# edwardyang12/Dex-NERF

Hardware: AMD Instinct MI355X
Metric: rays/sec (64+128 samples) + PSNR vs ref, 400x400 scene (higher is better)
Workload: dtype bf16; 1 GPU; C2 render: 400x400 rays/step/GPU, 64 coarse + 128 fine samples, coarse+fine FlexibleNeRFModel D8/W256/skip4 + viewdirs, PE L=10/4, 20 Dex thresholds, validation mode (det. resampling, no noise)

## Files before the change

### dex-nerf_amd/csrc/api.cpp

```cpp
#include <cstdlib>
#include <cstring>
#include <utility>
#include <vector>

#include "dn_common.h"
#include "composite_body.h"
#include "dn_rng.h"

namespace dn {

static thread_local char g_err[512] = "";

void set_error(const char* fmt, ...) {
  va_list ap;
  va_start(ap, fmt);
  vsnprintf(g_err, sizeof(g_err), fmt, ap);
  va_end(ap);
}

int ensure_big_lds(const void* kernel) {
  int dev = 0;
  if (hipGetDevice(&dev) != hipSuccess) dev = 0;
  static thread_local std::vector<std::pair<const void*, int>> done;
  for (const auto& kd : done)
    if (kd.first == kernel && kd.second == dev) return 0;
  hipError_t e = hipFuncSetAttribute(kernel, hipFuncAttributeMaxDynamicSharedMemorySize, 160 * 1024);
  if (e != hipSuccess) { set_error("hipFuncSetAttribute(device %d): %s", dev, hipGetErrorString(e)); return -static_cast<int>(e); }
  done.emplace_back(kernel, dev);
  return 0;
}

int device_cus() {
  constexpr int kMaxDev = 64;
  static thread_local int cache[kMaxDev] = {0};
  int dev = 0;
  if (hipGetDevice(&dev) != hipSuccess || dev < 0 || dev >= kMaxDev) return 256;
  if (cache[dev] == 0) {
    int cus = 256;
    if (hipDeviceGetAttribute(&cus, hipDeviceAttributeMultiprocessorCount, dev) != hipSuccess || cus <= 0) cus = 256;
    cache[dev] = cus;
  }
  return cache[dev];
}

static size_t align256(size_t v) { return (v + 255) & ~static_cast<size_t>(255); }

struct Workspace {
  float *z_c, *rf_c, *w_c, *z_f, *rf_f, *g_rf;
  unsigned* absmax_part;
  unsigned* status;
  size_t bytes;
};

static Workspace carve(void* base, int64_t n, int nc, int nf, bool train = false) {
  Workspace w{};
  size_t off = 0;
  auto take = [&](size_t floats) {
    float* p = base ? reinterpret_cast<float*>(static_cast<char*>(base) + off) : nullptr;
    off += align256(floats * sizeof(float));
    return p;
  };
  w.z_c = take(static_cast<size_t>(n) * nc);
  w.rf_c = take(static_cast<size_t>(n) * nc * 4);
  w.w_c = take(static_cast<size_t>(n) * nc);
  if (nf > 0) {
    w.z_f = take(static_cast<size_t>(n) * (nc + nf));
    w.rf_f = take(static_cast<size_t>(n) * (nc + nf) * 4);
  }
  if (train) w.g_rf = take(static_cast<size_t>(n) * (nc + nf) * 4);
  if (train) w.absmax_part = reinterpret_cast<unsigned*>(take(static_cast<size_t>((n + 3) / 4)));
  w.status = reinterpret_cast<unsigned*>(take(64));
  w.bytes = off;
  return w;
}

}

using namespace dn;

extern "C" int dn_abi_version(void) { return DN_ABI_VERSION; }

extern "C" const char* dn_last_error(void) { return g_err; }

extern "C" size_t dn_render_workspace_bytes(int64_t n_rays, int num_coarse, int num_fine) {
  if (n_rays < 0 || num_coarse < 1 || num_fine < 0) return 0;
  return carve(nullptr, n_rays, num_coarse, num_fine).bytes;
}

extern "C" int dn_render_rays(const dn_mlp_desc* desc_coarse, const void* packed_coarse, const dn_mlp_desc* desc_fine,
                              const void* packed_fine, int precision, const float* rays, int ray_stride,
                              int64_t n_rays, int num_coarse, int num_fine, int lindisp, float noise_std,
                              int white_background, const float* h_m_thres, int n_thres, const float* t_rand,
                              const float* noise_c, const float* u, const float* noise_f, float* rgb_c,
                              float* depth_c, float* acc_c, float* rgb_f, float* depth_f, float* acc_f, float* dex_f,
                              void* workspace, dn_stream_t stream) {
  if (n_rays == 0) return 0;
  DN_REQUIRE(desc_coarse && packed_coarse && rays && workspace && n_rays >= 0, "dn_render_rays: bad arguments");
  DN_REQUIRE(num_fine == 0 || (desc_fine && packed_fine), "dn_render_rays: fine pass requested without a fine net");
  DN_REQUIRE((reinterpret_cast<uintptr_t>(workspace) & 255) == 0, "dn_render_rays: workspace must be 256-byte aligned");
  if (n_rays == 0) return 0;
  Workspace w = carve(workspace, n_rays, num_coarse, num_fine);
  int rc;
  {
    hipError_t e = hipMemsetAsync(w.status, 0, 256, as_stream(stream));
    if (e != hipSuccess) { set_error("dn_render_rays: hipMemsetAsync: %s", hipGetErrorString(e)); return -static_cast<int>(e); }
  }
  if ((rc = dn_coarse_depths(rays, ray_stride, n_rays, num_coarse, lindisp, t_rand, w.z_c, stream))) return rc;
  const bool fine = num_fine > 0;
  DN_REQUIRE(n_thres >= 0 && n_thres <= kMaxThres, "dn_render_rays: at most %d Dex thresholds", kMaxThres);
  auto comp_for = [&](float* rgb, float* acc, float* weights, float* depth, float* dex, int k) {
    CompParams c{};
    c.rgb = rgb; c.acc = acc; c.weights = weights; c.depth = depth; c.dex = dex; c.disp = nullptr;
    c.nonfinite = w.status; c.n_rays = n_rays; c.n_thres = k; c.white = white_background;
    for (int i = 0; i < kMaxThres; ++i) c.th.m[i] = (i < k) ? h_m_thres[i] : 0.0f;
    return c;
  };
  const bool may_fuse = !(noise_std > 0.0f);
  int done = 0;
  {
    const CompParams c = comp_for(rgb_c, acc_c, w.w_c, depth_c, fine ? nullptr : dex_f, fine ? 0 : n_thres);
    if ((rc = run_network_flagged(desc_coarse, precision, packed_coarse, nullptr, nullptr, rays, ray_stride, w.z_c, n_rays,
                                  num_coarse, w.rf_c, w.status + 1, stream, (may_fuse && rgb_c) ? &c : nullptr, &done)))
      return rc;
  }
  if (!done && (rc = volume_render_counting(w.rf_c, w.z_c, rays + 3, ray_stride, noise_c, noise_std, white_background, h_m_thres,
                                            fine ? 0 : n_thres, n_rays, num_coarse, rgb_c, nullptr, acc_c, w.w_c, depth_c,
                                            fine ? nullptr : dex_f, w.status, stream)))
    return rc;
  if (!fine) return 0;
  if ((rc = dn_fine_depths(w.z_c, w.w_c, u, n_rays, num_coarse, num_fine, w.z_f, nullptr, stream))) return rc;
  {
    const CompParams c = comp_for(rgb_f, acc_f, nullptr, depth_f, dex_f, n_thres);
    if ((rc = run_network_flagged(desc_fine, precision, packed_fine, nullptr, nullptr, rays, ray_stride, w.z_f, n_rays,
                                  num_coarse + num_fine, w.rf_f, w.status + 1, stream, (may_fuse && rgb_f) ? &c : nullptr, &done)))
      return rc;
  }
  if (done) return 0;
  return volume_render_counting(w.rf_f, w.z_f, rays + 3, ray_stride, noise_f, noise_std, white_background, h_m_thres, n_thres,
                                n_rays, num_coarse + num_fine, rgb_f, nullptr, acc_f, nullptr, depth_f, dex_f, w.status, stream);
}

extern "C" size_t dn_render_train_workspace_bytes(int64_t n_rays, int num_coarse, int num_fine) {
  if (n_rays < 0 || num_coarse < 1 || num_fine < 0) return 0;
  return carve(nullptr, n_rays, num_coarse, num_fine, true).bytes;
}

extern "C" int dn_render_rays_train(const dn_mlp_desc* desc_coarse, const void* packed_coarse, const dn_mlp_desc* desc_fine,
                                    const void* packed_fine, int precision, const float* rays, int ray_stride,
                                    int64_t n_rays, int num_coarse, int num_fine, int lindisp, float noise_std,
                                    int white_background, const float* h_m_thres, int n_thres, const float* t_rand,
                                    const float* noise_c, const float* u, const float* noise_f, float* rgb_c,
                                    float* depth_c, float* acc_c, float* rgb_f, float* depth_f, float* acc_f, float* dex_f,
                                    void* workspace, void* act_c, void* masks_c, void* act_f, void* masks_f,
                                    const uint32_t* rng_state, int perturb, dn_stream_t stream) {
  if (n_rays == 0) return 0;
  DN_REQUIRE(desc_coarse && packed_coarse && rays && workspace && act_c && masks_c && n_rays >= 0, "dn_render_rays_train: bad arguments");
  DN_REQUIRE(num_fine == 0 || (desc_fine && packed_fine && act_f && masks_f), "dn_render_rays_train: fine pass requested without a fine net / its buffers");
  DN_REQUIRE((reinterpret_cast<uintptr_t>(workspace) & 255) == 0, "dn_render_rays_train: workspace must be 256-byte aligned");
  Workspace w = carve(workspace, n_rays, num_coarse, num_fine, true);
  int rc;
  const uint32_t* rng_perturb = perturb ? rng_state : nullptr;
  if ((rc = coarse_depths_rng(rays, ray_stride, n_rays, num_coarse, lindisp, t_rand, w.z_c, rng_perturb, stream))) return rc;
  if ((rc = dn_run_network_train(desc_coarse, precision, packed_coarse, nullptr, nullptr, rays, ray_stride, w.z_c, n_rays,
                                 num_coarse, w.rf_c, act_c, masks_c, stream)))
    return rc;
  const bool fine = num_fine > 0;
  if ((rc = volume_render_counting(w.rf_c, w.z_c, rays + 3, ray_stride, noise_c, noise_std, white_background, h_m_thres,
                                   fine ? 0 : n_thres, n_rays, num_coarse, rgb_c, nullptr, acc_c, w.w_c, depth_c,
                                   fine ? nullptr : dex_f, nullptr, stream, rng_state, kRngStreamNoiseCoarse)))
    return rc;
  if (!fine) return 0;
  if ((rc = fine_depths_rng(w.z_c, w.w_c, u, n_rays, num_coarse, num_fine, w.z_f, nullptr, rng_perturb, stream))) return rc;
  if ((rc = dn_run_network_train(desc_fine, precision, packed_fine, nullptr, nullptr, rays, ray_stride, w.z_f, n_rays,
                                 num_coarse + num_fine, w.rf_f, act_f, masks_f, stream)))
    return rc;
  return volume_render_counting(w.rf_f, w.z_f, rays + 3, ray_stride, noise_f, noise_std, white_background, h_m_thres, n_thres,
                                n_rays, num_coarse + num_fine, rgb_f, nullptr, acc_f, nullptr, depth_f, dex_f, nullptr, stream,
                                rng_state, kRngStreamNoiseFine);
}

extern "C" int dn_render_rays_backward_ws(const dn_mlp_desc* desc_coarse, const void* packed_bwd_coarse,
                                          const dn_mlp_desc* desc_fine, const void* packed_bwd_fine, int precision,
                                          const float* rays, int ray_stride, int64_t n_rays, int num_coarse, int num_fine,
                                          float noise_std, int white_background, const float* noise_c, const float* noise_f,
                                          const float* g_rgb_c, const float* g_depth_c, const float* g_acc_c,
                                          const float* g_rgb_f, const float* g_depth_f, const float* g_acc_f, void* workspace,
                                          const void* act_c, const void* masks_c, void* grads_c, const void* act_f,
                                          const void* masks_f, void* grads_f, float* const* h_dW_c, float* const* h_db_c,
                                          float* const* h_dW_f, float* const* h_db_f, int nets, const uint32_t* rng_state,
                                          void* wg_scratch, size_t wg_scratch_bytes, dn_stream_t stream) {
  if (n_rays == 0) return 0;
  DN_REQUIRE(rays && workspace && n_rays >= 0 && (nets & ~3) == 0 && (wg_scratch != nullptr || wg_scratch_bytes == 0), "dn_render_rays_backward: bad arguments");
  DN_REQUIRE((reinterpret_cast<uintptr_t>(workspace) & 255) == 0, "dn_render_rays_backward: workspace must be 256-byte aligned");
  Workspace w = carve(workspace, n_rays, num_coarse, num_fine, true);
  int rc;
  const bool pair_wgrad = nets == 3 && num_fine > 0 && desc_coarse && desc_fine && std::memcmp(desc_coarse, desc_fine, sizeof(dn_mlp_desc)) == 0 &&
                          weight_grad_pair_fits(*desc_fine);
  auto half = [&](const dn_mlp_desc* desc, const void* packed_bwd, const float* rf, const float* z, int samples,
                  const float* noise, const float* g_rgb, const float* g_depth, const float* g_acc, const void* act,
                  const void* masks, void* grads, float* const* h_dW, float* const* h_db, uint32_t noise_stream) -> int {
    DN_REQUIRE(desc && packed_bwd && act && masks && grads && h_dW && h_db, "dn_render_rays_backward: a network's buffers are missing");
    const int64_t n_parts = (n_rays + 3) / 4;
    unsigned* parts = (precision == DN_PREC_BF16_S8 && s8_scale_is_per_launch() && n_parts <= 4096 && std::getenv("DEXNERF_S8_ABSMAX_KERNEL") == nullptr)
                          ? w.absmax_part : nullptr;
    if ((rc = volume_render_backward_rng(rf, z, rays + 3, ray_stride, noise, noise_std, white_background, n_rays, samples,
                                         g_rgb, g_depth, g_acc, nullptr, nullptr, w.g_rf, rng_state, noise_stream, stream, parts)))
      return rc;
    const int64_t n_points = n_rays * samples;
    if ((rc = mlp_backward_data_partials(desc, precision, packed_bwd, w.g_rf, masks, n_points, grads, parts, static_cast<int>(parts ? n_parts : 0), stream))) return rc;
    if (pair_wgrad) return 0;
    return dn_mlp_weight_grad_all_ws(desc, precision, act, grads, n_points, h_dW, h_db, wg_scratch, wg_scratch_bytes, stream);
  };
  if ((nets & 2) && num_fine > 0) {
    if ((rc = half(desc_fine, packed_bwd_fine, w.rf_f, w.z_f, num_coarse + num_fine, noise_f, g_rgb_f, g_depth_f, g_acc_f,
                   act_f, masks_f, grads_f, h_dW_f, h_db_f, kRngStreamNoiseFine)))
      return rc;
  }
  if (nets & 1) {
    if ((rc = half(desc_coarse, packed_bwd_coarse, w.rf_c, w.z_c, num_coarse, noise_c, g_rgb_c, g_depth_c, g_acc_c, act_c,
                   masks_c, grads_c, h_dW_c, h_db_c, kRngStreamNoiseCoarse)))
      return rc;
  }
  if (pair_wgrad)
    return dn_mlp_weight_grad_pair_ws(desc_fine, precision, act_f, grads_f, n_rays * (num_coarse + num_fine), h_dW_f, h_db_f, act_c, grads_c,
                                      n_rays * num_coarse, h_dW_c, h_db_c, wg_scratch, wg_scratch_bytes, stream);
  return 0;
}

extern "C" int dn_render_rays_backward(const dn_mlp_desc* desc_coarse, const void* packed_bwd_coarse,
                                       const dn_mlp_desc* desc_fine, const void* packed_bwd_fine, int precision,
                                       const float* rays, int ray_stride, int64_t n_rays, int num_coarse, int num_fine,
                                       float noise_std, int white_background, const float* noise_c, const float* noise_f,
                                       const float* g_rgb_c, const float* g_depth_c, const float* g_acc_c,
                                       const float* g_rgb_f, const float* g_depth_f, const float* g_acc_f, void* workspace,
                                       const void* act_c, const void* masks_c, void* grads_c, const void* act_f,
                                       const void* masks_f, void* grads_f, float* const* h_dW_c, float* const* h_db_c,
                                       float* const* h_dW_f, float* const* h_db_f, int nets, const uint32_t* rng_state,
                                       dn_stream_t stream) {
  return dn_render_rays_backward_ws(desc_coarse, packed_bwd_coarse, desc_fine, packed_bwd_fine, precision, rays, ray_stride, n_rays, num_coarse,
                                    num_fine, noise_std, white_background, noise_c, noise_f, g_rgb_c, g_depth_c, g_acc_c, g_rgb_f, g_depth_f,
                                    g_acc_f, workspace, act_c, masks_c, grads_c, act_f, masks_f, grads_f, h_dW_c, h_db_c, h_dW_f, h_db_f, nets,
                                    rng_state, nullptr, 0, stream);
}
```

### dex-nerf_amd/csrc/dn_common.h

```cpp
#pragma once
#include <hip/hip_runtime.h>
#include <cstdarg>
#include <cstdint>
#include <cstdio>

#include "../../include/dexnerf_hip.h"

namespace dn {

constexpr int kWave = 64;

void set_error(const char* fmt, ...);

inline hipStream_t as_stream(dn_stream_t s) { return reinterpret_cast<hipStream_t>(s); }

inline int check_launch(const char* what) {
  hipError_t e = hipGetLastError();
  if (e != hipSuccess) {
    set_error("%s: %s", what, hipGetErrorString(e));
    return -static_cast<int>(e);
  }
  return 0;
}

int ensure_big_lds(const void* kernel);
int device_cus();

int volume_render_counting(const float* rf, const float* z, const float* rd, int rd_stride, const float* noise, float noise_std,
                           int white_background, const float* h_m_thres, int n_thres, int64_t n_rays, int n_samples, float* rgb,
                           float* disp, float* acc, float* weights, float* depth, float* dex, unsigned* nonfinite,
                           dn_stream_t stream, const uint32_t* rng_state = nullptr, uint32_t rng_stream = 0);

bool weight_grad_pair_fits(const dn_mlp_desc& d);
struct CompParams;
int run_network_flagged(const dn_mlp_desc* desc, int precision, const void* packed, const float* pts, const float* viewdirs,
                        const float* rays, int ray_stride, const float* z_vals, int64_t n_rays, int samples_per_ray, float* out,
                        unsigned* range_flag, dn_stream_t stream, const CompParams* comp = nullptr, int* composited = nullptr);

int coarse_depths_rng(const float* rays, int ray_stride, int64_t n_rays, int num_coarse, int lindisp, const float* t_rand,
                      float* z_vals, const uint32_t* rng_state, dn_stream_t stream);
int fine_depths_rng(const float* z_coarse, const float* weights, const float* u, int64_t n_rays, int num_coarse, int num_fine,
                    float* z_fine, float* z_samples, const uint32_t* rng_state, dn_stream_t stream);
int volume_render_backward_rng(const float* rf, const float* z, const float* rd, int rd_stride, const float* noise, float noise_std,
                               int white_background, int64_t n_rays, int n_samples, const float* g_rgb, const float* g_depth,
                               const float* g_acc, const float* g_disp, const float* g_weights, float* g_rf,
                               const uint32_t* rng_state, uint32_t rng_stream, dn_stream_t stream, unsigned* absmax_part = nullptr);
int mlp_backward_data_partials(const dn_mlp_desc* desc, int precision, const void* packed_bwd, const float* g_out, const void* masks,
                               int64_t n_points, void* grads, const unsigned* partials, int n_partials, dn_stream_t stream);
bool s8_scale_is_per_launch();

#define DN_REQUIRE(cond, ...)     \
  do {                            \
    if (!(cond)) {                \
      dn::set_error(__VA_ARGS__); \
      return DN_E_INVAL;          \
    }                             \
  } while (0)

__device__ __forceinline__ int lane_id() { return threadIdx.x & 63; }

template <int CTRL>
__device__ __forceinline__ unsigned dpp_bits(unsigned v) {
  return static_cast<unsigned>(__builtin_amdgcn_update_dpp(0, static_cast<int>(v), CTRL, 0xF, 0xF, false));
}
constexpr int kDppXor1 = 0xB1, kDppXor2 = 0x4E, kDppHalfMirror = 0x141, kDppMirror = 0x140;

template <class Op>
__device__ __forceinline__ float wave_allreduce(float v, Op op) {
  auto f = [](unsigned b) { return __builtin_bit_cast(float, b); };
  auto u = [](float x) { return __builtin_bit_cast(unsigned, x); };
  v = op(v, f(dpp_bits<kDppXor1>(u(v))));
  v = op(v, f(dpp_bits<kDppXor2>(u(v))));
  v = op(v, f(dpp_bits<kDppHalfMirror>(u(v))));
  v = op(v, f(dpp_bits<kDppMirror>(u(v))));
  { const auto r = __builtin_amdgcn_permlane16_swap(u(v), u(v), false, false); v = op(f(r[0]), f(r[1])); }
  { const auto r = __builtin_amdgcn_permlane32_swap(u(v), u(v), false, false); v = op(f(r[0]), f(r[1])); }
  return v;
}

__device__ __forceinline__ float wave_sum(float v) { return wave_allreduce(v, [](float a, float b) { return a + b; }); }
__device__ __forceinline__ float wave_max(float v) { return wave_allreduce(v, [](float a, float b) { return fmaxf(a, b); }); }

__device__ __forceinline__ double wave_sum(double v) {
  auto mv = [](double x, auto step) {
    const unsigned long long b = __builtin_bit_cast(unsigned long long, x);
    const unsigned lo = step(static_cast<unsigned>(b)), hi = step(static_cast<unsigned>(b >> 32));
    return __builtin_bit_cast(double, (static_cast<unsigned long long>(hi) << 32) | lo);
  };
  v += mv(v, [](unsigned w) { return dpp_bits<kDppXor1>(w); });
  v += mv(v, [](unsigned w) { return dpp_bits<kDppXor2>(w); });
  v += mv(v, [](unsigned w) { return dpp_bits<kDppHalfMirror>(w); });
  v += mv(v, [](unsigned w) { return dpp_bits<kDppMirror>(w); });
  {
    const unsigned long long b = __builtin_bit_cast(unsigned long long, v);
    const auto lo = __builtin_amdgcn_permlane16_swap(static_cast<unsigned>(b), static_cast<unsigned>(b), false, false);
    const auto hi = __builtin_amdgcn_permlane16_swap(static_cast<unsigned>(b >> 32), static_cast<unsigned>(b >> 32), false, false);
    v = __builtin_bit_cast(double, (static_cast<unsigned long long>(hi[0]) << 32) | lo[0]) +
        __builtin_bit_cast(double, (static_cast<unsigned long long>(hi[1]) << 32) | lo[1]);
  }
  {
    const unsigned long long b = __builtin_bit_cast(unsigned long long, v);
    const auto lo = __builtin_amdgcn_permlane32_swap(static_cast<unsigned>(b), static_cast<unsigned>(b), false, false);
    const auto hi = __builtin_amdgcn_permlane32_swap(static_cast<unsigned>(b >> 32), static_cast<unsigned>(b >> 32), false, false);
    v = __builtin_bit_cast(double, (static_cast<unsigned long long>(hi[0]) << 32) | lo[0]) +
        __builtin_bit_cast(double, (static_cast<unsigned long long>(hi[1]) << 32) | lo[1]);
  }
  return v;
}

template <int CTRL, int ROW_MASK>
__device__ __forceinline__ double dpp_or_one(double v) {
  const unsigned long long b = __builtin_bit_cast(unsigned long long, v);
  const unsigned lo = static_cast<unsigned>(__builtin_amdgcn_update_dpp(0, static_cast<int>(static_cast<unsigned>(b)), CTRL, ROW_MASK, 0xF, false));
  const unsigned hi = static_cast<unsigned>(__builtin_amdgcn_update_dpp(0x3FF00000, static_cast<int>(static_cast<unsigned>(b >> 32)), CTRL, ROW_MASK, 0xF, false));
  return __builtin_bit_cast(double, (static_cast<unsigned long long>(hi) << 32) | lo);
}
__device__ __forceinline__ double wave_scan_mul(double v) {
  v *= dpp_or_one<0x111, 0xF>(v);
  v *= dpp_or_one<0x112, 0xF>(v);
  v *= dpp_or_one<0x114, 0xF>(v);
  v *= dpp_or_one<0x118, 0xF>(v);
  v *= dpp_or_one<0x142, 0xA>(v);
  v *= dpp_or_one<0x143, 0xC>(v);
  return v;
}
__device__ __forceinline__ double wave_shift_up1(double v, double first) {
  const unsigned long long b = __builtin_bit_cast(unsigned long long, v), f = __builtin_bit_cast(unsigned long long, first);
  const unsigned lo = static_cast<unsigned>(__builtin_amdgcn_update_dpp(static_cast<int>(static_cast<unsigned>(f)), static_cast<int>(static_cast<unsigned>(b)), 0x138, 0xF, 0xF, false));
  const unsigned hi = static_cast<unsigned>(__builtin_amdgcn_update_dpp(static_cast<int>(static_cast<unsigned>(f >> 32)), static_cast<int>(static_cast<unsigned>(b >> 32)), 0x138, 0xF, 0xF, false));
  return __builtin_bit_cast(double, (static_cast<unsigned long long>(hi) << 32) | lo);
}
__device__ __forceinline__ double wave_last(double v) {
  const unsigned long long b = __builtin_bit_cast(unsigned long long, v);
  const unsigned lo = static_cast<unsigned>(__builtin_amdgcn_readlane(static_cast<int>(static_cast<unsigned>(b)), 63));
  const unsigned hi = static_cast<unsigned>(__builtin_amdgcn_readlane(static_cast<int>(static_cast<unsigned>(b >> 32)), 63));
  return __builtin_bit_cast(double, (static_cast<unsigned long long>(hi) << 32) | lo);
}

__device__ __forceinline__ double wave_scan_add(double v) {
  const int l = lane_id();
#pragma unroll
  for (int o = 1; o < 64; o <<= 1) {
    double t = __shfl_up(v, o, 64);
    if (l >= o) v += t;
  }
  return v;
}

__device__ __forceinline__ float wave_scan_add(float v) {
  const int l = lane_id();
#pragma unroll
  for (int o = 1; o < 64; o <<= 1) {
    float t = __shfl_up(v, o, 64);
    if (l >= o) v += t;
  }
  return v;
}

__host__ __device__ __forceinline__ float linspace_elem(float start, float end, int steps, int i) {
  if (steps == 1) return start;
  const float step = (end - start) / static_cast<float>(steps - 1);
  return (i < steps / 2) ? fmaf(step, static_cast<float>(i), start)
                         : fmaf(-step, static_cast<float>(steps - 1 - i), end);
}

}
```

### dex-nerf_amd/csrc/mlp_device.h

```cpp
#pragma once
#include <cstdlib>
#include <utility>

#include "mlp_layout.h"

namespace dn {

typedef float f32x16 __attribute__((ext_vector_type(16)));
typedef float f32x4 __attribute__((ext_vector_type(4)));
typedef __bf16 bf16x8 __attribute__((ext_vector_type(8)));
typedef _Float16 f16x8 __attribute__((ext_vector_type(8)));

template <int N, class F, int... I>
__device__ __forceinline__ void static_for_impl(F&& f, std::integer_sequence<int, I...>) {
  (f(std::integral_constant<int, I>{}), ...);
}
template <int N, class F>
__device__ __forceinline__ void static_for(F&& f) {
  static_for_impl<N>(static_cast<F&&>(f), std::make_integer_sequence<int, N>{});
}

constexpr int kRingPhases = 5;
constexpr int kSlotBytes = kPhasePieces * kPieceBytes;
constexpr int kRingBytes = kRingPhases * kSlotBytes;
constexpr int kInRows = 10;

template <int BF16> struct Prec;
template <> struct Prec<1> {
  using BPiece = bf16x8;
  using Elem = __bf16;
  static constexpr int EPP = 8;
  static constexpr int PPT = 2;
};
template <> struct Prec<2> {
  using BPiece = f16x8;
  using Elem = _Float16;
  static constexpr int EPP = 8;
  static constexpr int PPT = 2;
};
template <> struct Prec<0> {
  using BPiece = f32x4;
  using Elem = float;
  static constexpr int EPP = 4;
  static constexpr int PPT = 4;
};
template <int BF16, int PT> constexpr int waves_of() { return (BF16 && PT == 1) ? 8 : 4; }

struct FwdParams {
  const char* packed;
  int bias_bytes;
  int total_pieces;
  int D;
  unsigned skip_mask;
  int use_viewdirs;
  int mode;
  const float* rays;
  int ray_stride;
  const float* z;
  const float* pts;
  const float* viewdirs;
  const float* enc;
  int enc_ld;
  long long n_points;
  int S;
  long long n_tiles;
  float* out;
  float fx[16];
  float fd[8];
  char* act;
  char* masks;
  int act_pieces, mask_words;
  int slot_xyz, slot_dir, slot_layer1, slot_trunk0, slot_feat, slot_dirout;
  int save8;
  unsigned* range_flag;
};

template <bool ASM_READS_, bool LEADER_DMA_, bool SCALAR_STATE_, int PREFETCH_>
struct PipeGeometry {
  static constexpr bool ASM_READS = ASM_READS_, LEADER_DMA = LEADER_DMA_, SCALAR_STATE = SCALAR_STATE_;
  static constexpr int PREFETCH = PREFETCH_;
};
template <int WAVES, class G>
struct PipeT {
  static constexpr int PER_WAVE = kPhasePieces / WAVES;
  char* ring;
  unsigned ring_addr;
  const char* wsrc;
  unsigned total_bytes;
  unsigned q_issue;
  unsigned slot_wr, slot_nxt;
  unsigned wave;
  unsigned pend_src, pend_dst;
  const char* rd_cur;
  const char* rd_nxt;
  unsigned lane16;
  f32x4 af[G::PREFETCH];
  unsigned rda_cur;
  unsigned slot_cur_base;
  f32x4 bias_nxt;

  __device__ __forceinline__ void dma_phase(unsigned src_off, unsigned dst_off, unsigned go) {
    const unsigned long long src_bits = reinterpret_cast<unsigned long long>(wsrc + src_off);
    const unsigned lo = __builtin_amdgcn_readfirstlane(static_cast<unsigned>(src_bits));
    const unsigned hi = __builtin_amdgcn_readfirstlane(static_cast<unsigned>(src_bits >> 32));
    const char* src = reinterpret_cast<const char*>((static_cast<unsigned long long>(hi) << 32) | lo);
    const unsigned lds = __builtin_amdgcn_readfirstlane(ring_addr + dst_off);
    go = __builtin_amdgcn_readfirstlane(go);
    unsigned keep;
    if constexpr (PER_WAVE == 2) {
      asm volatile(
          "s_cmp_lg_u32 %[go], 0\n\t"
          "s_cbranch_scc0 .Ldn_dma_skip%=\n\t"
          "s_mov_b32 %[keep], m0\n\t"
          "s_mov_b32 m0, %[lds]\n\t"
          "s_nop 1\n\t"
          "global_load_lds_dwordx4 %[voff], %[sbase]\n\t"
          "global_load_lds_dwordx4 %[voff], %[sbase] offset:1024\n\t"
          "s_mov_b32 m0, %[keep]\n"
          ".Ldn_dma_skip%=:"
          : [keep] "=&s"(keep)
          : [go] "s"(go), [lds] "s"(lds), [voff] "v"(lane16), [sbase] "s"(src)
          : "memory", "scc");
    } else {
      asm volatile(
          "s_cmp_lg_u32 %[go], 0\n\t"
          "s_cbranch_scc0 .Ldn_dma_skip%=\n\t"
          "s_mov_b32 %[keep], m0\n\t"
          "s_mov_b32 m0, %[lds]\n\t"
          "s_nop 1\n\t"
          "global_load_lds_dwordx4 %[voff], %[sbase]\n\t"
          "global_load_lds_dwordx4 %[voff], %[sbase] offset:1024\n\t"
          "global_load_lds_dwordx4 %[voff], %[sbase] offset:2048\n\t"
          "global_load_lds_dwordx4 %[voff], %[sbase] offset:3072\n\t"
          "s_mov_b32 m0, %[keep]\n"
          ".Ldn_dma_skip%=:"
          : [keep] "=&s"(keep)
          : [go] "s"(go), [lds] "s"(lds), [voff] "v"(lane16), [sbase] "s"(src)
          : "memory", "scc");
    }
  }

  __device__ __forceinline__ void advance_issue() {
    const unsigned who = wave;
    if constexpr (G::LEADER_DMA) {
      pend_src = q_issue + who * (2 * PER_WAVE * kPieceBytes);
      pend_dst = slot_wr * kSlotBytes + who * (2 * PER_WAVE * kPieceBytes);
    } else {
      pend_src = q_issue + who * (PER_WAVE * kPieceBytes);
      pend_dst = slot_wr * kSlotBytes + who * (PER_WAVE * kPieceBytes);
    }
    q_issue += kSlotBytes;
    if (q_issue >= total_bytes) q_issue = 0;
    slot_wr = (slot_wr + 1 == kRingPhases) ? 0 : slot_wr + 1;
    if constexpr (G::SCALAR_STATE) {
      q_issue = __builtin_amdgcn_readfirstlane(q_issue);
      slot_wr = __builtin_amdgcn_readfirstlane(slot_wr);
      pend_src = __builtin_amdgcn_readfirstlane(pend_src);
      pend_dst = __builtin_amdgcn_readfirstlane(pend_dst);
    }
  }

  __device__ __forceinline__ void issue_phase() {
    advance_issue();
    if constexpr (G::LEADER_DMA) {
      dma_phase(pend_src, pend_dst, wave < 4 ? 1u : 0u);
      dma_phase(pend_src + PER_WAVE * kPieceBytes, pend_dst + PER_WAVE * kPieceBytes, wave < 4 ? 1u : 0u);
    } else {
      dma_phase(pend_src, pend_dst, 1u);
    }
  }

  __device__ __forceinline__ void phase_begin() {
    static_assert(kRingPhases == 5, "the counted waits below assume two younger phases in flight");
    if constexpr (G::ASM_READS) {
      static_assert(!G::ASM_READS || PER_WAVE == 2, "the asm-read pipeline is the 8-wave geometry");
      if constexpr (G::LEADER_DMA) asm volatile("s_waitcnt vmcnt(8)" ::: "memory");
      else asm volatile("s_waitcnt vmcnt(4)" ::: "memory");
    } else {
      if constexpr (PER_WAVE == 2) asm volatile("s_waitcnt vmcnt(4) lgkmcnt(0)" ::: "memory");
      else asm volatile("s_waitcnt vmcnt(8) lgkmcnt(0)" ::: "memory");
    }
    __builtin_amdgcn_s_barrier();
    advance_issue();
    dma_phase(pend_src, pend_dst, (WAVES == 4 || wave < 4) ? 1u : 0u);
    slot_nxt = (slot_nxt + 1 == kRingPhases) ? 0 : slot_nxt + 1;
    if constexpr (G::ASM_READS) {
      rda_cur = slot_cur_base + lane16;
      slot_cur_base = __builtin_amdgcn_readfirstlane(ring_addr + slot_nxt * kSlotBytes);
    } else {
      rd_cur = rd_nxt;
      rd_nxt = ring + slot_nxt * kSlotBytes + lane16;
    }
  }

  __device__ __forceinline__ void mid_phase() {
    if constexpr (WAVES == 8 && G::LEADER_DMA) dma_phase(pend_src + PER_WAVE * kPieceBytes, pend_dst + PER_WAVE * kPieceBytes, wave < 4 ? 1u : 0u);
    else if constexpr (WAVES == 8) dma_phase(pend_src, pend_dst, wave >= 4 ? 1u : 0u);
  }

  template <bool EVEN>
  __device__ __forceinline__ void phase_begin2() {
    if constexpr (EVEN) {
      asm volatile("s_waitcnt vmcnt(0)" ::: "memory");
      __builtin_amdgcn_s_barrier();
      advance_issue();
      dma_phase(pend_src, pend_dst, wave < 4 ? 1u : 0u);
      dma_phase(pend_src + PER_WAVE * kPieceBytes, pend_dst + PER_WAVE * kPieceBytes, wave < 4 ? 1u : 0u);
    }
    slot_nxt = (slot_nxt + 1 == kRingPhases) ? 0 : slot_nxt + 1;
    rda_cur = slot_cur_base + lane16;
    slot_cur_base = __builtin_amdgcn_readfirstlane(ring_addr + slot_nxt * kSlotBytes);
  }
  template <bool EVEN>
  __device__ __forceinline__ void mid_phase2() {
    if constexpr (EVEN) {
      advance_issue();
      dma_phase(pend_src, pend_dst, wave < 4 ? 1u : 0u);
      dma_phase(pend_src + PER_WAVE * kPieceBytes, pend_dst + PER_WAVE * kPieceBytes, wave < 4 ? 1u : 0u);
    }
  }
  unsigned long long xs_src[2];
  unsigned xs_dst[2];
  template <int PERIOD>
  __device__ __forceinline__ void xs_period_begin() {
    static_assert(PERIOD == kPhasePieces || PERIOD == 2 * kPhasePieces, "barrier period: one or two phases");
    if constexpr (PERIOD == 2 * kPhasePieces) asm volatile("s_waitcnt vmcnt(0)" ::: "memory");
    else asm volatile("s_waitcnt vmcnt(8)" ::: "memory");
    __builtin_amdgcn_s_barrier();
#pragma unroll
    for (int h = 0; h < PERIOD / kPhasePieces; ++h) {
      advance_issue();
      const unsigned long long bits = reinterpret_cast<unsigned long long>(wsrc + pend_src);
      const unsigned lo = __builtin_amdgcn_readfirstlane(static_cast<unsigned>(bits));
      const unsigned hi = __builtin_amdgcn_readfirstlane(static_cast<unsigned>(bits >> 32));
      xs_src[h] = (static_cast<unsigned long long>(hi) << 32) | lo;
      xs_dst[h] = __builtin_amdgcn_readfirstlane(ring_addr + pend_dst);
    }
  }
  template <int PERIOD, int Q>
  __device__ __forceinline__ void xs_dma_step() {
    constexpr int STEPS = PERIOD / 8;
    constexpr int H = (Q % STEPS) / 2;
    constexpr int OFF = (Q % 2) * 2048;
    unsigned keep;
    asm volatile(
        "s_cmp_lg_u32 %[wave], %[who]\n\t"
        "s_cbranch_scc1 .Ldn_xs_skip%=\n\t"
        "s_mov_b32 %[keep], m0\n\t"
        "s_mov_b32 m0, %[lds]\n\t"
        "s_nop 1\n\t"
        "global_load_lds_dwordx4 %[voff], %[sbase] offset:%[o0]\n\t"
        "global_load_lds_dwordx4 %[voff], %[sbase] offset:%[o1]\n\t"
        "s_mov_b32 m0, %[keep]\n"
        ".Ldn_xs_skip%=:"
        : [keep] "=&s"(keep)
        : [wave] "s"(wave), [who] "n"(Q / STEPS), [lds] "s"(xs_dst[H]), [voff] "v"(lane16), [sbase] "s"(xs_src[H]), [o0] "n"(OFF), [o1] "n"(OFF + 1024)
        : "memory", "scc");
  }
  template <int PERIOD, int POS>
  __device__ __forceinline__ void at_position_xs() {
    if constexpr (POS % PERIOD == 0) xs_period_begin<PERIOD>();
    if constexpr (POS % kPhasePieces == 0) {
      slot_nxt = (slot_nxt + 1 == kRingPhases) ? 0 : slot_nxt + 1;
      rda_cur = slot_cur_base + lane16;
      slot_cur_base = __builtin_amdgcn_readfirstlane(ring_addr + slot_nxt * kSlotBytes);
    }
  }
  template <int PERIOD, int POS>
  __device__ __forceinline__ void xs_after_piece() {
    if constexpr ((POS % PERIOD) < PERIOD / 2) xs_dma_step<PERIOD, POS % PERIOD>();
  }
  template <int PH, int POS>
  __device__ __forceinline__ void at_position() {
    static_assert(PH == kPhasePieces || (G::ASM_READS && G::LEADER_DMA), "the two-phase barrier period is the 48-point geometry's");
    if constexpr (POS % kPhasePieces == 0) {
      if constexpr (PH == 2 * kPhasePieces) phase_begin2<(POS % PH) == 0>();
      else phase_begin();
    }
    if constexpr (POS % kPhasePieces == kPhasePieces / 2) {
      if constexpr (PH == 2 * kPhasePieces) mid_phase2<(POS % PH) == kPhasePieces / 2>();
      else mid_phase();
    }
  }

  template <int POS, int N, int PH = kPhasePieces, bool BIAS = true>
  __device__ __forceinline__ void skip() {
    static_for<N>([&](auto i_c) {
      constexpr int pos = POS + decltype(i_c)::value;
      static_assert(pos % kPhasePieces != 0 || decltype(i_c)::value == 0, "padding never crosses a phase");
      if constexpr (pos % kPhasePieces == kPhasePieces / 2) at_position<PH, pos>();
      if constexpr (!G::ASM_READS || decltype(i_c)::value >= N - G::PREFETCH) prefetch<pos>();
    });
    settle<BIAS>();
  }

  template <int PERIOD, int POS, int N>
  __device__ __forceinline__ void skip_xs() {
    static_for<N>([&](auto i_c) {
      constexpr int pos = POS + decltype(i_c)::value;
      static_assert(pos % kPhasePieces != 0 || decltype(i_c)::value == 0, "padding never crosses a phase");
      static_assert(pos % PERIOD != 0, "padding never opens a barrier period");
      xs_after_piece<PERIOD, pos>();
      if constexpr (decltype(i_c)::value >= N - G::PREFETCH) prefetch<pos>();
    });
    settle<true>();
  }

  template <int POS>
  __device__ __forceinline__ void prefetch() {
    constexpr int q = (POS % kPhasePieces) + G::PREFETCH;
    if constexpr (G::ASM_READS) {
      const unsigned base = (q < kPhasePieces) ? rda_cur : slot_cur_base + lane16;
      asm volatile("ds_read_b128 %0, %1 offset:%2" : "=v"(af[POS % G::PREFETCH]) : "v"(base), "n"((q % kPhasePieces) * kPieceBytes));
    } else {
      const char* base = (q < kPhasePieces) ? rd_cur : rd_nxt;
      af[POS % G::PREFETCH] = *reinterpret_cast<const f32x4*>(base + (q % kPhasePieces) * kPieceBytes);
    }
  }

  template <int E>
  __device__ __forceinline__ void prologue_read() {
    asm volatile("ds_read_b128 %0, %1 offset:%2" : "=v"(af[E]) : "v"(slot_cur_base + lane16), "n"(E * kPieceBytes));
  }
  template <int POS, int NEWER>
  __device__ __forceinline__ f32x4 take() {
    asm volatile("s_waitcnt lgkmcnt(%1)" : "+v"(af[POS % G::PREFETCH]) : "n"(NEWER));
    return af[POS % G::PREFETCH];
  }
  template <int OFF>
  __device__ __forceinline__ void bias_prefetch(unsigned addr) {
    asm volatile("ds_read_b128 %0, %1 offset:%2" : "=v"(bias_nxt) : "v"(addr), "n"(OFF));
  }
  template <int NEWER>
  __device__ __forceinline__ f32x4 bias_take() {
    asm volatile("s_waitcnt lgkmcnt(%1)" : "+v"(bias_nxt) : "n"(NEWER));
    return bias_nxt;
  }
  template <bool BIAS = true>
  __device__ __forceinline__ void settle() {
    if constexpr (!G::ASM_READS) return;
    static_assert(G::PREFETCH >= 2 && G::PREFETCH <= 4, "settle() names every FIFO entry");
    if constexpr (!BIAS) {
      static_assert(G::PREFETCH == 2, "the bias-less form is the 48-point pipeline's");
      asm volatile("s_waitcnt lgkmcnt(0)" : "+v"(af[0]), "+v"(af[1]));
    } else
    if constexpr (G::PREFETCH == 2) asm volatile("s_waitcnt lgkmcnt(0)" : "+v"(af[0]), "+v"(af[1]), "+v"(bias_nxt));
    else if constexpr (G::PREFETCH == 3) asm volatile("s_waitcnt lgkmcnt(0)" : "+v"(af[0]), "+v"(af[1]), "+v"(af[2]), "+v"(bias_nxt));
    else asm volatile("s_waitcnt lgkmcnt(0)" : "+v"(af[0]), "+v"(af[1]), "+v"(af[2]), "+v"(af[G::PREFETCH - 1]), "+v"(bias_nxt));
  }
};
using PipeGeo32 = PipeGeometry<false, false, false, 4>;
template <int WAVES>
using Pipe = PipeT<WAVES, PipeGeo32>;

template <int BF16>
__device__ __forceinline__ f32x16 mma_piece(f32x16 acc, f32x4 a_raw, typename Prec<BF16>::BPiece b) {
  if constexpr (BF16 == 1) {
    const bf16x8 a = __builtin_bit_cast(bf16x8, a_raw);
    return __builtin_amdgcn_mfma_f32_32x32x16_bf16(a, b, acc, 0, 0, 0);
  } else if constexpr (BF16 == 2) {
    const f16x8 a = __builtin_bit_cast(f16x8, a_raw);
    return __builtin_amdgcn_mfma_f32_32x32x16_f16(a, b, acc, 0, 0, 0);
  } else {
    acc = __builtin_amdgcn_mfma_f32_32x32x2f32(a_raw[0], b[0], acc, 0, 0, 0);
    acc = __builtin_amdgcn_mfma_f32_32x32x2f32(a_raw[1], b[1], acc, 0, 0, 0);
    acc = __builtin_amdgcn_mfma_f32_32x32x2f32(a_raw[2], b[2], acc, 0, 0, 0);
    acc = __builtin_amdgcn_mfma_f32_32x32x2f32(a_raw[3], b[3], acc, 0, 0, 0);
    return acc;
  }
}

template <int BF16, int PT, int NT_OUT, int KH, int KP, int POS0, bool HAS_BIAS = true, class PipeT, class BH, class BP, class Emit>
__device__ __forceinline__ void run_stage(PipeT& pipe, const BH& bh , BP&& bp ,
                                          const char* bias_lds , Emit&& emit) {
  constexpr int KT = KH + KP;
  static_for<NT_OUT>([&](auto nt_c) {
    constexpr int nt = decltype(nt_c)::value;
    f32x4 b0 = {0.f, 0.f, 0.f, 0.f}, b1 = b0, b2 = b0, b3 = b0;
    if constexpr (HAS_BIAS) {
      const f32x4* bptr = reinterpret_cast<const f32x4*>(bias_lds + nt * 128);
      b0 = bptr[0]; b1 = bptr[1]; b2 = bptr[2]; b3 = bptr[3];
    }
    f32x16 a[PT];
#pragma unroll
    for (int t = 0; t < PT; ++t) {
      a[t][0] = b0[0]; a[t][1] = b0[1]; a[t][2] = b0[2]; a[t][3] = b0[3];
      a[t][4] = b1[0]; a[t][5] = b1[1]; a[t][6] = b1[2]; a[t][7] = b1[3];
      a[t][8] = b2[0]; a[t][9] = b2[1]; a[t][10] = b2[2]; a[t][11] = b2[3];
      a[t][12] = b3[0]; a[t][13] = b3[1]; a[t][14] = b3[2]; a[t][15] = b3[3];
    }
    static_for<KT>([&](auto k_c) {
      constexpr int k = decltype(k_c)::value;
      constexpr int pos = POS0 + nt * KT + k;
      if constexpr (pos % kPhasePieces == 0) pipe.phase_begin();
      if constexpr (pos % kPhasePieces == kPhasePieces / 2) pipe.mid_phase();
      const f32x4 araw = pipe.af[pos % PipeGeo32::PREFETCH];
      static_for<PT>([&](auto t_c) {
        constexpr int t = decltype(t_c)::value;
        if constexpr (k < KH) a[t] = mma_piece<BF16>(a[t], araw, bh[t][k]);
        else a[t] = mma_piece<BF16>(a[t], araw, bp(t, k - KH));
      });
      pipe.template prefetch<pos>();
      __builtin_amdgcn_sched_group_barrier(0x008, (BF16 ? 1 : 4) * PT, 0);
      __builtin_amdgcn_sched_group_barrier(0x100, 1, 0);
    });
    __builtin_amdgcn_sched_barrier(0);
    static_for<PT>([&](auto t_c) { emit(nt_c, t_c, a[decltype(t_c)::value]); });
  });
}

template <int BF16, bool RELU, int S>
__device__ __forceinline__ typename Prec<BF16>::BPiece make_piece(const f32x16& acc) {
  using P = Prec<BF16>;
  typename P::BPiece piece;
  if constexpr (BF16) {
#pragma unroll
    for (int e = 0; e < 8; ++e) piece[e] = static_cast<typename P::Elem>(acc[S * 8 + e]);
    if constexpr (RELU) {
      typedef short s16x8 __attribute__((ext_vector_type(8)));
      s16x8 bits = __builtin_bit_cast(s16x8, piece);
      const s16x8 zero = {0, 0, 0, 0, 0, 0, 0, 0};
      bits = __builtin_elementwise_max(bits, zero);
      piece = __builtin_bit_cast(typename P::BPiece, bits);
    }
  } else {
#pragma unroll
    for (int e = 0; e < 4; ++e) piece[e] = RELU ? fmaxf(acc[S * 4 + e], 0.0f) : acc[S * 4 + e];
  }
  return piece;
}

template <int BF16, bool RELU, int NT, class BO>
__device__ __forceinline__ void emit_pieces(const f32x16& acc, BO& bo) {
  using P = Prec<BF16>;
  static_for<P::PPT>([&](auto s_c) {
    constexpr int s = decltype(s_c)::value;
    bo[NT * P::PPT + s] = make_piece<BF16, RELU, s>(acc);
  });
}

__device__ __forceinline__ const char* uniform_ptr(const char* p) {
  const unsigned long long bits = reinterpret_cast<unsigned long long>(p);
  const unsigned lo = __builtin_amdgcn_readfirstlane(static_cast<unsigned>(bits));
  const unsigned hi = __builtin_amdgcn_readfirstlane(static_cast<unsigned>(bits >> 32));
  return reinterpret_cast<const char*>((static_cast<unsigned long long>(hi) << 32) | lo);
}

template <class V>
__device__ __forceinline__ void store16_uniform(const char* base, unsigned lane16, const V& val) {
  static_assert(sizeof(V) == 16, "one dwordx4 per lane");
  const char* b = uniform_ptr(base);
  const unsigned voff = lane16;
  const f32x4 data = __builtin_bit_cast(f32x4, val);
#define DN_STORE_POLICY " nt"
  asm volatile("s_nop 4\n\tglobal_store_dwordx4 %[voff], %[data], %[sbase]" DN_STORE_POLICY "\n\ts_nop 1"
               : : [voff] "v"(voff), [data] "v"(data), [sbase] "s"(b) : "memory");
}

template <class V>
__device__ __forceinline__ void store16_uniform_at(const char* base, unsigned byte_off, unsigned lane16, const V& val) {
  static_assert(sizeof(V) == 16, "one dwordx4 per lane");
  const char* b = base;
  const unsigned off = byte_off;
  const unsigned voff = lane16;
  const f32x4 data = __builtin_bit_cast(f32x4, val);
  unsigned tmp;
  asm volatile("v_add_u32 %[tmp], %[off], %[voff]\n\ts_nop 4\n\tglobal_store_dwordx4 %[tmp], %[data], %[sbase]" DN_STORE_POLICY "\n\ts_nop 1"
               : [tmp] "=&v"(tmp) : [voff] "v"(voff), [off] "s"(off), [data] "v"(data), [sbase] "s"(b) : "memory");
}

template <class V>
__device__ __forceinline__ void store16_unit48(const char* base, unsigned byte_off, unsigned lane16, const V& val) {
  static_assert(sizeof(V) == 16, "one dwordx4 per lane");
  const char* b = base;
  const unsigned off = byte_off;
  const unsigned voff = lane16;
  const f32x4 data = __builtin_bit_cast(f32x4, val);
  unsigned tmp;
  asm volatile("v_and_b32 %[tmp], 0x100, %[voff]\n\tv_lshrrev_b32 %[tmp], 1, %[tmp]\n\tv_xor_b32 %[tmp], %[tmp], %[voff]\n\tv_add_u32 %[tmp], %[off], %[tmp]\n\t"
               "s_nop 0\n\tglobal_store_dwordx4 %[tmp], %[data], %[sbase]" DN_STORE_POLICY "\n\ts_nop 1"
               : [tmp] "=&v"(tmp) : [voff] "v"(voff), [off] "s"(off), [data] "v"(data), [sbase] "s"(b) : "memory");
}

constexpr float kE4m3Max = 448.0f, kE5m2Max = 57344.0f;
template <bool GRAD>
__device__ __forceinline__ void piece_to_8bit(const bf16x8& v, float scale, unsigned& w0, unsigned& w1) {
  float f[8];
#pragma unroll
  for (int e = 0; e < 8; ++e) {
    f[e] = static_cast<float>(v[e]);
    if constexpr (GRAD) f[e] = __builtin_amdgcn_fmed3f(f[e] * scale, -kE5m2Max, kE5m2Max);
    else f[e] = __builtin_amdgcn_fmed3f(f[e], -kE4m3Max, kE4m3Max);
  }
  int a = 0, b = 0;
  if constexpr (GRAD) {
    a = __builtin_amdgcn_cvt_pk_bf8_f32(f[0], f[1], a, false); a = __builtin_amdgcn_cvt_pk_bf8_f32(f[2], f[3], a, true);
    b = __builtin_amdgcn_cvt_pk_bf8_f32(f[4], f[5], b, false); b = __builtin_amdgcn_cvt_pk_bf8_f32(f[6], f[7], b, true);
  } else {
    a = __builtin_amdgcn_cvt_pk_fp8_f32(f[0], f[1], a, false); a = __builtin_amdgcn_cvt_pk_fp8_f32(f[2], f[3], a, true);
    b = __builtin_amdgcn_cvt_pk_fp8_f32(f[4], f[5], b, false); b = __builtin_amdgcn_cvt_pk_fp8_f32(f[6], f[7], b, true);
  }
  w0 = static_cast<unsigned>(a); w1 = static_cast<unsigned>(b);
}

__device__ __forceinline__ void dma16_lanes(const void* src_lane, unsigned lds_addr) {
  const unsigned lds = __builtin_amdgcn_readfirstlane(lds_addr);
  const void* src = src_lane;
  unsigned keep;
  asm volatile(
      "s_mov_b32 %[keep], m0\n\t"
      "s_mov_b32 m0, %[lds]\n\t"
      "s_nop 1\n\t"
      "global_load_lds_dwordx4 %[vaddr], off\n\t"
      "s_mov_b32 m0, %[keep]"
      : [keep] "=&s"(keep)
      : [lds] "s"(lds), [vaddr] "v"(src)
      : "memory");
}

template <bool BF8>
__device__ __forceinline__ unsigned cvt_pairs_8bit(unsigned d0, unsigned d1, float scale) {
  unsigned r;
  if constexpr (BF8)
    asm("v_cvt_scalef32_pk_bf8_bf16 %0, %1, %3\n\tv_cvt_scalef32_pk_bf8_bf16 %0, %2, %3 op_sel:[0,0,1]" : "=&v"(r) : "v"(d0), "v"(d1), "v"(scale));
  else
    asm("v_cvt_scalef32_pk_fp8_bf16 %0, %1, %3\n\tv_cvt_scalef32_pk_fp8_bf16 %0, %2, %3 op_sel:[0,0,1]" : "=&v"(r) : "v"(d0), "v"(d1), "v"(scale));
  return r;
}

__device__ __forceinline__ void dma4_lanes48(const void* src_lane, unsigned lds_addr) {
  const unsigned lds = __builtin_amdgcn_readfirstlane(lds_addr);
  const void* src = src_lane;
  unsigned keep;
  asm volatile(
      "s_mov_b32 %[keep], m0\n\t"
      "s_mov_b32 m0, %[lds]\n\t"
      "s_mov_b32 exec_hi, 0xffff\n\t"
      "s_nop 1\n\t"
      "global_load_lds_dword %[vaddr], off\n\t"
      "s_mov_b32 exec_hi, -1\n\t"
      "s_mov_b32 m0, %[keep]"
      : [keep] "=&s"(keep)
      : [lds] "s"(lds), [vaddr] "v"(src)
      : "memory");
}

template <int BF16, int L, int NPIECES, class BP>
__device__ __forceinline__ void encode_pieces(const float (&x)[3], const float* freqs, int h, BP& bp) {
  using P = Prec<BF16>;
  constexpr int NF = L / 2;
  float sv[NF][3], cv[NF][3];
#pragma unroll
  for (int f = 0; f < NF; ++f) {
    const float fr = h ? freqs[NF + f] : freqs[f];
#pragma unroll
    for (int c = 0; c < 3; ++c) {
      const float arg = x[c] * fr;
      if constexpr (BF16) {
        const float rev = __builtin_amdgcn_fractf(arg * 0.15915494309189535f);
        sv[f][c] = __builtin_amdgcn_sinf(rev);
        cv[f][c] = __builtin_amdgcn_cosf(rev);
      } else {
        sincosf(arg, &sv[f][c], &cv[f][c]);
      }
    }
  }
  static_for<NPIECES>([&](auto p_c) {
    constexpr int p = decltype(p_c)::value;
    typename P::BPiece piece;
    static_for<P::EPP>([&](auto e_c) {
      constexpr int e = decltype(e_c)::value;
      constexpr int u = p * P::EPP + e;
      float v;
      if constexpr (u < 6 * NF) v = ((u % 6) < 3) ? sv[u / 6][u % 3] : cv[u / 6][u % 3];
      else if constexpr (u == 6 * NF) v = h ? x[2] : x[0];
      else if constexpr (u == 6 * NF + 1) v = h ? 0.0f : x[1];
      else v = 0.0f;
      piece[e] = static_cast<typename P::Elem>(v);
    });
    bp[p] = piece;
  });
}

template <int BF16, int L, int NPIECES, class BP>
__device__ __forceinline__ void gather_pieces(const float* row, int h, BP& bp) {
  using P = Prec<BF16>;
  static_for<NPIECES>([&](auto p_c) {
    constexpr int p = decltype(p_c)::value;
    typename P::BPiece piece;
#pragma unroll
    for (int e = 0; e < P::EPP; ++e) {
      const int col = pe_slot_col(L, h, p * P::EPP + e);
      const float v = (col >= 0) ? row[col] : 0.0f;
      piece[e] = static_cast<typename P::Elem>(v);
    }
    bp[p] = piece;
  });
}

}
```

### dex-nerf_amd/csrc/mlp_fused.hip

```cpp
#include "mlp_fused_kernel.h"
#include "mlp_internal.h"
#include "mlp_geo48.h"

namespace dn {

DN_FWD32_INSTANCES(DN_FWD32_EXTERN)


template <int BF16>
__global__ void pack_kernel(NetLayout L, PackPtrs ptrs, char* __restrict__ packed) {
  using P = Prec<BF16>;
  const int KX = kXyzPanel, KD = round_up(3 + 6 * L.LD, 16);
  (void)KX; (void)KD;
  const int n_bias = L.total_bias_tiles * 32;
  float* bias_out = reinterpret_cast<float*>(packed);
  for (int idx = blockIdx.x * blockDim.x + threadIdx.x; idx < L.bias_bytes / 4; idx += gridDim.x * blockDim.x) {
    float v = 0.0f;
    if (idx < n_bias) {
      const int tile = idx / 32, hh = (idx % 32) / 16, r = idx % 16;
      int s = 0;
      while (s + 1 < L.n_stages && L.st[s + 1].bias0 <= tile) ++s;
      const StageDesc& st = L.st[s];
      int ts = tile - st.bias0;
      const int row_in_tile = acc_row(r, hh);
      if (st.src2 >= 0) {
        if (ts == 0) v = (row_in_tile == 0) ? ptrs.b[st.src2][0] : 0.0f;
        else { const int n = (ts - 1) * 32 + row_in_tile; v = (n < st.n_real) ? ptrs.b[st.src][n] : 0.0f; }
      } else {
        const int n = ts * 32 + row_in_tile;
        v = (n < st.n_real) ? ptrs.b[st.src][n] : 0.0f;
      }
    }
    bias_out[idx] = v;
  }
  char* wout = packed + L.bias_bytes;
  const long long n_elems = static_cast<long long>(L.total_pieces) * 64 * P::EPP;
  for (long long idx = static_cast<long long>(blockIdx.x) * blockDim.x + threadIdx.x; idx < n_elems;
       idx += static_cast<long long>(gridDim.x) * blockDim.x) {
    const int e = static_cast<int>(idx % P::EPP);
    const int lane = static_cast<int>((idx / P::EPP) % 64);
    const int piece = static_cast<int>(idx / (P::EPP * 64));
    const int i = lane & 31, hh = lane >> 5;
    float v = 0.0f;
    int s = 0;
    while (s + 1 < L.n_stages && L.st[s + 1].piece0 <= piece) ++s;
    const StageDesc& st = L.st[s];
    const int rel = piece - st.piece0;
    if (st.transposed) {
      if (rel < st.n_tiles * st.pieces_per_tile) {
        const int ts = rel / st.pieces_per_tile;
        const int k = rel % st.pieces_per_tile;
        const int kh = st.hidden_in / (2 * P::EPP);
        const int row = ts * 32 + i;
        if (row < st.n_real) {
          if (k < kh) {
            const int kout = (k / P::PPT) * 32 + acc_row((k % P::PPT) * P::EPP + e, hh);
            v = ptrs.w[st.src][static_cast<long long>(kout) * st.ld + st.col_hidden0 + row];
          } else {
            const int kc = hh * P::EPP + e;
            if (kc < st.custom_k) {
              const int srcw = st.src2 >= 0 ? st.src2 : st.src;
              v = ptrs.w[srcw][static_cast<long long>(kc) * st.ld + st.col_hidden0 + row];
            }
          }
        }
      }
    } else if (rel < st.n_tiles * st.pieces_per_tile) {
      const int ts = rel / st.pieces_per_tile;
      const int k = rel % st.pieces_per_tile;
      const int kh = st.hidden_in / (2 * P::EPP);
      int col;
      if (k < kh) {
        const int nt_in = k / P::PPT;
        const int r = (k % P::PPT) * P::EPP + e;
        col = st.col_hidden0 + nt_in * 32 + acc_row(r, hh);
      } else {
        const int u = (k - kh) * P::EPP + e;
        const int pc = pe_slot_col(st.pe_kind == 1 ? L.LX : L.LD, hh, u);
        col = (pc >= 0) ? st.col_pe0 + pc : -1;
      }
      if (col >= 0) {
        if (st.src2 >= 0) {
          if (ts == 0) v = (i == 0) ? ptrs.w[st.src2][col] : 0.0f;
          else { const int n = (ts - 1) * 32 + i; v = (n < st.n_real) ? ptrs.w[st.src][static_cast<long long>(n) * st.ld + col] : 0.0f; }
        } else {
          const int n = ts * 32 + i;
          v = (n < st.n_real) ? ptrs.w[st.src][static_cast<long long>(n) * st.ld + col] : 0.0f;
        }
      }
    }
    reinterpret_cast<typename P::Elem*>(wout)[idx] = static_cast<typename P::Elem>(v);
  }
}

template <int W, int LX, int LD, int BF16, int PT, int SAVE>
static int launch_forward(FwdParams p, hipStream_t stream) {
  auto kern = mlp_forward_kernel<W, LX, LD, BF16, PT, SAVE>;
  constexpr int WAVES = waves_of<BF16, PT>();
  constexpr int PTS_PER_WG = WAVES * 32 * PT;
  constexpr int KXP = kXyzPanel / (2 * Prec<BF16>::EPP);
  p.n_tiles = (p.n_points + PTS_PER_WG - 1) / PTS_PER_WG;
  constexpr int KDP = round_up(3 + 6 * LD, 16) / (2 * Prec<BF16>::EPP);
  const size_t lds = kRingBytes + p.bias_bytes + WAVES * (kInRows * 32 * PT * sizeof(float) + PT * (KXP + KDP) * kPieceBytes);
  if (int rc = ensure_big_lds(reinterpret_cast<const void*>(kern))) return rc;
  const int cus = device_cus();
  const long long grid = p.n_tiles < cus ? p.n_tiles : cus;
  hipLaunchKernelGGL(kern, dim3(static_cast<unsigned>(grid)), dim3(WAVES * 64), lds, stream, p);
  return check_launch("mlp_forward");
}

int dispatch_forward(const dn_mlp_desc& d, int precision, FwdParams& p, hipStream_t stream, const CompParams* comp, int* composited) {
  const bool bf = precision == DN_PREC_BF16;
  const bool hf = precision == DN_PREC_F16;
  const char* geom_env = getenv("DEXNERF_BF16_GEOM");
  const bool geom48 = !(geom_env && atoi(geom_env) == 32);
  if ((bf || hf) && geom48 && p.act == nullptr && p.mode != 2 && p.n_points < (1LL << 31) - 1024 && g48_supported(d, precision))
    return launch_forward48(d, precision, p, p.packed + p.bias_bytes + static_cast<size_t>(p.total_pieces) * kPieceBytes, stream, comp, composited);
  if (p.act != nullptr && hf) { set_error("mlp_forward(train): fp16 is a render-only mode"); return DN_E_UNSUPPORTED; }
  if (p.act != nullptr && p.save8) {
    if (!bf || p.mode == 2 || !g48_train_supported(d) || p.n_points >= (1LL << 31) - 1024) {
      set_error("mlp_forward(train, 8-bit saved tensors): bf16 arithmetic, rays / points input, W in {128, 256}, L_xyz in {6, 10}, a depth the 48-point kernel holds in LDS");
      return DN_E_UNSUPPORTED;
    }
    return launch_forward48(d, precision, p, p.packed + p.bias_bytes + static_cast<size_t>(p.total_pieces) * kPieceBytes, stream);
  }
  const int prec_arg = bf ? 1 : hf ? 2 : 0;
  const int save = p.act != nullptr ? 1 : 0;
#define DN_CASE(W_, LX_, F_, SAVE_)                                                            \
  if (d.hidden_size == W_ && d.num_encoding_fn_xyz == LX_ && prec_arg == F_ && save == SAVE_) \
    return launch_forward<W_, LX_, 4, F_, 1, SAVE_>(p, stream);
  DN_FWD32_INSTANCES(DN_CASE)
#undef DN_CASE
  if (save) {
    set_error("mlp_forward(train): no kernel instance for W=%d L_xyz=%d", d.hidden_size, d.num_encoding_fn_xyz);
    return DN_E_UNSUPPORTED;
  }
  if (hf) {
    set_error("mlp_forward(fp16): no kernel instance for W=%d L_xyz=%d", d.hidden_size, d.num_encoding_fn_xyz);
    return DN_E_UNSUPPORTED;
  }
  set_error("mlp_forward: no kernel instance for W=%d L_xyz=%d", d.hidden_size, d.num_encoding_fn_xyz);
  return DN_E_UNSUPPORTED;
}

void fill_freqs(float* f, int num_fns, int log_sampling);

int setup_params(const dn_mlp_desc* desc, int precision, const void* packed, FwdParams* p) {
  int rc = validate_desc(desc, precision);
  if (rc) return rc;
  NetLayout L;
  build_layout(*desc, precision, &L);
  *p = FwdParams{};
  p->packed = static_cast<const char*>(packed);
  p->bias_bytes = L.bias_bytes;
  p->total_pieces = L.total_pieces;
  p->D = desc->num_layers;
  p->skip_mask = L.skip_mask;
  p->use_viewdirs = desc->use_viewdirs;
  fill_freqs(p->fx, desc->num_encoding_fn_xyz, desc->log_sampling_xyz);
  if (desc->use_viewdirs) fill_freqs(p->fd, desc->num_encoding_fn_dir, desc->log_sampling_dir);
  return 0;
}

int launch_pack(const NetLayout& L, const PackPtrs& ptrs, void* packed, int precision, hipStream_t stream) {
  if (precision == DN_PREC_BF16)
    hipLaunchKernelGGL(pack_kernel<1>, dim3(512), dim3(256), 0, stream, L, ptrs, static_cast<char*>(packed));
  else if (precision == DN_PREC_F16)
    hipLaunchKernelGGL(pack_kernel<2>, dim3(512), dim3(256), 0, stream, L, ptrs, static_cast<char*>(packed));
  else
    hipLaunchKernelGGL(pack_kernel<0>, dim3(512), dim3(256), 0, stream, L, ptrs, static_cast<char*>(packed));
  return check_launch("mlp_pack");
}

}

using namespace dn;

extern "C" size_t dn_mlp_packed_bytes(const dn_mlp_desc* desc, int precision) {
  if (validate_desc(desc, precision)) return 0;
  NetLayout L;
  build_layout(*desc, precision, &L);
  return static_cast<size_t>(L.bias_bytes) + static_cast<size_t>(L.total_pieces) * kPieceBytes +
         (g48_supported(*desc, precision) ? g48_region_bytes(*desc) : 0);
}

extern "C" int dn_fp16_range_guard(const dn_mlp_desc* desc) {
  if (validate_desc(desc, DN_PREC_F16)) return 0;
  return (std::getenv("DEXNERF_G48_RUNTIME_SHAPE") == nullptr && std::getenv("DEXNERF_BF16_GEOM") == nullptr && g48_range_guard_complete(*desc)) ? 1 : 0;
}

extern "C" int dn_mlp_pack(const dn_mlp_desc* desc, int precision, const float* const* h_weights,
                           const float* const* h_biases, void* packed, dn_stream_t stream) {
  return dn_mlp_pack_parts(desc, precision, h_weights, h_biases, packed, DN_PACK_ALL, stream);
}

extern "C" int dn_mlp_pack_parts(const dn_mlp_desc* desc, int precision, const float* const* h_weights,
                                 const float* const* h_biases, void* packed, int parts, dn_stream_t stream) {
  int rc = validate_desc(desc, precision);
  if (rc) return rc;
  DN_REQUIRE(h_weights && h_biases && packed, "dn_mlp_pack: NULL pointer");
  DN_REQUIRE(parts != 0 && (parts & ~DN_PACK_ALL) == 0, "dn_mlp_pack_parts: parts must be a non-empty mask of DN_PACK_CORE | DN_PACK_G48");
  DN_REQUIRE((reinterpret_cast<uintptr_t>(packed) & 15) == 0, "dn_mlp_pack: packed buffer must be 16-byte aligned");
  NetLayout L;
  build_layout(*desc, precision, &L);
  const int n_params = desc->num_layers + (desc->use_viewdirs ? 4 : 1);
  PackPtrs ptrs{};
  for (int i = 0; i < n_params; ++i) {
    DN_REQUIRE(h_weights[i] && h_biases[i], "dn_mlp_pack: parameter %d is NULL", i);
    ptrs.w[i] = h_weights[i];
    ptrs.b[i] = h_biases[i];
  }
  if (parts & DN_PACK_CORE) rc = launch_pack(L, ptrs, packed, precision, as_stream(stream));
  if (rc == 0 && (parts & DN_PACK_G48) && g48_supported(*desc, precision))
    rc = launch_pack48(*desc, precision, ptrs, static_cast<char*>(packed) + L.bias_bytes + static_cast<size_t>(L.total_pieces) * kPieceBytes,
                       as_stream(stream));
  return rc;
}

extern "C" int dn_run_network(const dn_mlp_desc* desc, int precision, const void* packed, const float* pts,
                              const float* viewdirs, const float* rays, int ray_stride, const float* z_vals,
                              int64_t n_rays, int samples_per_ray, float* out, dn_stream_t stream) {
  return dn::run_network_flagged(desc, precision, packed, pts, viewdirs, rays, ray_stride, z_vals, n_rays, samples_per_ray, out,
                                 nullptr, stream);
}

int dn::run_network_flagged(const dn_mlp_desc* desc, int precision, const void* packed, const float* pts,
                            const float* viewdirs, const float* rays, int ray_stride, const float* z_vals,
                            int64_t n_rays, int samples_per_ray, float* out, unsigned* range_flag, dn_stream_t stream,
                            const CompParams* comp, int* composited) {
  if (composited) *composited = 0;
  FwdParams p;
  int rc = setup_params(desc, precision, packed, &p);
  if (rc) return rc;
  if (n_rays == 0) return 0;
  DN_REQUIRE(packed && out && n_rays >= 0 && samples_per_ray >= 1, "dn_run_network: bad arguments");
  DN_REQUIRE((reinterpret_cast<uintptr_t>(out) & 15) == 0, "dn_run_network: out must be 16-byte aligned");
  if (pts != nullptr) {
    DN_REQUIRE(!desc->use_viewdirs || viewdirs, "dn_run_network: viewdirs required with use_viewdirs");
    p.mode = 1; p.pts = pts; p.viewdirs = viewdirs;
  } else {
    DN_REQUIRE(rays && z_vals, "dn_run_network: need pts, or rays + z_vals");
    DN_REQUIRE(ray_stride >= (desc->use_viewdirs ? 11 : 8), "dn_run_network: ray_stride too small");
    p.mode = 0; p.rays = rays; p.ray_stride = ray_stride; p.z = z_vals;
  }
  p.n_points = n_rays * samples_per_ray;
  p.S = samples_per_ray;
  p.out = out;
  p.range_flag = range_flag;
  if (p.n_points == 0) return 0;
  return dispatch_forward(*desc, precision, p, as_stream(stream), comp, composited);
}

extern "C" int dn_mlp_forward_encoded(const dn_mlp_desc* desc, int precision, const void* packed, const float* x,
                                      int64_t n_rows, float* out, dn_stream_t stream) {
  FwdParams p;
  int rc = setup_params(desc, precision, packed, &p);
  if (rc) return rc;
  if (n_rows == 0) return 0;
  DN_REQUIRE(packed && x && out && n_rows >= 0, "dn_mlp_forward_encoded: bad arguments");
  DN_REQUIRE((reinterpret_cast<uintptr_t>(out) & 15) == 0, "dn_mlp_forward_encoded: out must be 16-byte aligned");
  p.mode = 2; p.enc = x;
  p.enc_ld = (3 + 6 * desc->num_encoding_fn_xyz) + (desc->use_viewdirs ? 3 + 6 * desc->num_encoding_fn_dir : 0);
  p.n_points = n_rows; p.S = 1; p.out = out;
  if (n_rows == 0) return 0;
  return dispatch_forward(*desc, precision, p, as_stream(stream));
}
```

### dex-nerf_amd/csrc/mlp_fused48.hip

```cpp
#include "mlp_fused48_kernel.h"

namespace dn {

DN_FWD48_PAPER_BF16(DN_FWD48_EXTERN)
DN_FWD48_PAPER_FP16(DN_FWD48_EXTERN)
DN_FWD48_W128(DN_FWD48_EXTERN)
DN_FWD48_HOST_UNIT(DN_FWD48_INSTANTIATE)

template <int F>
__device__ __forceinline__ void pack48_body(const NetLayout& L, const PackPtrs& ptrs, const G48Tables& tabs, char* __restrict__ region);

template <int F>
__global__ void pack48_kernel(NetLayout L, PackPtrs ptrs, G48Tables tabs, char* __restrict__ region) {
  pack48_body<F>(L, ptrs, tabs, region);
}

template <int F>
__global__ void pack48_pair_kernel(NetLayout L, PackPtrs ptrs_a, PackPtrs ptrs_b, G48Tables tabs, char* __restrict__ region_a,
                                   char* __restrict__ region_b) {
  if (blockIdx.y == 0) pack48_body<F>(L, ptrs_a, tabs, region_a);
  else pack48_body<F>(L, ptrs_b, tabs, region_b);
}

template <int F>
__device__ __forceinline__ void pack48_body(const NetLayout& L, const PackPtrs& ptrs, const G48Tables& tabs, char* __restrict__ region) {
  using Elem = typename Prec<F>::Elem;
  const int n_rows = L.total_bias_tiles * 16;
  float* bias_out = reinterpret_cast<float*>(region);
  for (int idx = blockIdx.x * blockDim.x + threadIdx.x; idx < L.bias_bytes / 4; idx += gridDim.x * blockDim.x) {
    float v = 0.0f;
    if (idx < n_rows) {
      const int tile = idx / 16, r = idx % 16;
      int s = 0;
      while (s + 1 < L.n_stages && L.st[s + 1].bias0 <= tile) ++s;
      const StageDesc& st = L.st[s];
      const int ts = tile - st.bias0;
      if (st.src2 >= 0) {
        if (ts == 0) v = (r == 0) ? ptrs.b[st.src2][0] : 0.0f;
        else { const int n = (ts - 1) * 16 + r; v = (n < st.n_real) ? ptrs.b[st.src][n] : 0.0f; }
      } else {
        const int n = ts * 16 + r;
        v = (n < st.n_real) ? ptrs.b[st.src][n] : 0.0f;
      }
    }
    bias_out[idx] = v;
  }
  f32x4* tab = reinterpret_cast<f32x4*>(region + L.bias_bytes);
  for (int idx = blockIdx.x * blockDim.x + threadIdx.x; idx < kG48TableBytes / 16; idx += gridDim.x * blockDim.x) {
    const int kind_pe = idx < 64 ? 1 : 2;
    const int gg = idx < 64 ? idx / 16 : (idx - 64) / 8, u = idx < 64 ? idx % 16 : (idx - 64) % 8;
    const int c = g48_pe_col(kind_pe, gg, u, kind_pe == 1 ? L.LX : L.LD);
    f32x4 entry = {0.0f, 0.0f, 0.0f, 0.0f};
    if (c >= 0 && c < 3) entry[2] = 1.0f;
    else if (c >= 3) {
      const int qq = c - 3, f = qq / 6, r = qq % 6;
      entry[0] = (kind_pe == 1 ? tabs.fx[f] : tabs.fd[f]) * 0.15915494309189535f;
      entry[1] = r < 3 ? 0.0f : 0.25f;
      entry[3] = 1.0f;
    }
    tab[idx] = entry;
  }
  Elem* wout = reinterpret_cast<Elem*>(region + L.bias_bytes + kG48TableBytes);
  const long long n_elems = static_cast<long long>(L.total_pieces) * 64 * 8;
  for (long long idx = static_cast<long long>(blockIdx.x) * blockDim.x + threadIdx.x; idx < n_elems;
       idx += static_cast<long long>(gridDim.x) * blockDim.x) {
    const int e = static_cast<int>(idx % 8);
    const int lane = static_cast<int>((idx / 8) % 64);
    const int piece = static_cast<int>(idx / 512);
    const int i = lane & 15, gg = lane >> 4;
    float v = 0.0f;
    int s = 0;
    while (s + 1 < L.n_stages && L.st[s + 1].piece0 <= piece) ++s;
    const StageDesc& st = L.st[s];
    const int rel = piece - st.piece0;
    if (rel < st.n_tiles * st.pieces_per_tile) {
      const int ts = rel / st.pieces_per_tile;
      const int k = rel % st.pieces_per_tile;
      const int kh = st.hidden_in / 32;
      int col;
      if (k < kh) {
        col = st.col_hidden0 + g48_hidden_col(k, gg, e);
      } else {
        const int pc = g48_pe_col(st.pe_kind, gg, (k - kh) * 8 + e, st.pe_kind == 1 ? L.LX : L.LD);
        col = pc >= 0 ? st.col_pe0 + pc : -1;
      }
      if (col >= 0) {
        if (st.src2 >= 0) {
          if (ts == 0) v = (i == 0) ? ptrs.w[st.src2][col] : 0.0f;
          else { const int n = (ts - 1) * 16 + i; v = (n < st.n_real) ? ptrs.w[st.src][static_cast<long long>(n) * st.ld + col] : 0.0f; }
        } else {
          const int n = ts * 16 + i;
          v = (n < st.n_real) ? ptrs.w[st.src][static_cast<long long>(n) * st.ld + col] : 0.0f;
        }
      }
    }
    wout[idx] = static_cast<Elem>(v);
  }
}

void fill_freqs(float* f, int num_fns, int log_sampling);

int launch_pack48(const dn_mlp_desc& d, int precision, const PackPtrs& ptrs, char* region, hipStream_t stream) {
  NetLayout L;
  build_layout48(d, &L);
  G48Tables tabs{};
  fill_freqs(tabs.fx, d.num_encoding_fn_xyz, d.log_sampling_xyz);
  if (d.use_viewdirs) fill_freqs(tabs.fd, d.num_encoding_fn_dir, d.log_sampling_dir);
  tabs.LX = d.num_encoding_fn_xyz; tabs.LD = d.num_encoding_fn_dir;
  if (precision == DN_PREC_F16) hipLaunchKernelGGL(pack48_kernel<2>, dim3(pack48_blocks(L)), dim3(256), 0, stream, L, ptrs, tabs, region);
  else hipLaunchKernelGGL(pack48_kernel<1>, dim3(pack48_blocks(L)), dim3(256), 0, stream, L, ptrs, tabs, region);
  return check_launch("mlp_pack48");
}

bool g48_range_guard_complete(const dn_mlp_desc& d) {
  if (!g48_supported(d, DN_PREC_F16)) return false;
  NetLayout L;
  build_layout48(d, &L);
  const bool paper = d.hidden_size == 256 && d.num_layers == 8 && L.skip_mask == 0x10u && d.use_viewdirs;
  return paper || d.hidden_size == 128;
}

int launch_pack48_pair(const dn_mlp_desc& d, const PackPtrs& a, const PackPtrs& b, char* region_a, char* region_b, hipStream_t stream) {
  NetLayout L;
  build_layout48(d, &L);
  G48Tables tabs{};
  fill_freqs(tabs.fx, d.num_encoding_fn_xyz, d.log_sampling_xyz);
  if (d.use_viewdirs) fill_freqs(tabs.fd, d.num_encoding_fn_dir, d.log_sampling_dir);
  tabs.LX = d.num_encoding_fn_xyz; tabs.LD = d.num_encoding_fn_dir;
  static_assert(sizeof(NetLayout) + 2 * sizeof(PackPtrs) + sizeof(G48Tables) + 16 <= 4096, "kernel arguments of the pair pack");
  hipLaunchKernelGGL(pack48_pair_kernel<1>, dim3(pack48_blocks(L), 2), dim3(256), 0, stream, L, a, b, tabs, region_a, region_b);
  return check_launch("mlp_pack48_pair");
}

static bool fused_composite_enabled() {
  const char* e = std::getenv("DEXNERF_FUSED_COMPOSITE");
  return e != nullptr && std::atoi(e) == 1;
}

int launch_forward48(const dn_mlp_desc& d, int precision, const FwdParams& p_in, const char* region, hipStream_t stream,
                     const CompParams* comp, int* composited) {
  if (composited) *composited = 0;
  NetLayout L;
  build_layout48(d, &L);
  FwdParams p = p_in;
  G48Params q{};
  q.base = region; q.bias_bytes = L.bias_bytes; q.total_pieces = L.total_pieces;
  p.n_tiles = (p.n_points + kG48PointsPerWg - 1) / kG48PointsPerWg;
  size_t lds = g48_lds_bytes(L);
  if (lds > 160 * 1024) { set_error("mlp_forward48: %zu bytes of LDS", lds); return DN_E_UNSUPPORTED; }
  const int cus = device_cus();
  long long grid = p.n_tiles < cus ? p.n_tiles : cus;
  auto launch = [&](auto kern) -> int {
    if (int rc = ensure_big_lds(reinterpret_cast<const void*>(kern))) return rc;
    hipLaunchKernelGGL(kern, dim3(static_cast<unsigned>(grid)), dim3(kG48Waves * 64), lds, stream, p, q);
    return check_launch("mlp_forward48");
  };
  const bool paper = d.hidden_size == 256 && d.num_layers == 8 && L.skip_mask == 0x10u && d.use_viewdirs;
  const bool shipped = d.hidden_size == 128 && d.num_layers == 4 && L.skip_mask == 0u && d.use_viewdirs;
  const bool fixed_ok = std::getenv("DEXNERF_G48_RUNTIME_SHAPE") == nullptr;
  if (p.act != nullptr) {
    if (precision != DN_PREC_BF16 || !p.save8) { set_error("mlp_forward48(train): the 48-point training forward is the bf16 / 8-bit-saved-tensor mode"); return DN_E_UNSUPPORTED; }
    if (g48_two_group_shape(d) && g48_train_groups(p.n_points, cus) == 2) {
      p.n_tiles = (p.n_points + 255) / 256;
      grid = p.n_tiles < cus ? p.n_tiles : cus;
      return paper ? launch(mlp_forward48_kernel<256, 1, 8, 0x10u, 1, 3>) : launch(mlp_forward48_kernel<128, 1, 4, 0u, 1, 3>);
    }
    if (paper && fixed_ok) return launch(mlp_forward48_kernel<256, 1, 8, 0x10u, 1, 2>);
    if (shipped && fixed_ok) return launch(mlp_forward48_kernel<128, 1, 4, 0u, 1, 2>);
    return d.hidden_size == 256 ? launch(mlp_forward48_kernel<256, 1, 0, 0u, 0, 2>) : launch(mlp_forward48_kernel<128, 1, 0, 0u, 0, 2>);
  }
  if (comp != nullptr && comp->rgb != nullptr && (paper || shipped) && fixed_ok && p.mode == 0 && p.act == nullptr && p.S >= 1 &&
      kG48PointsPerWg % p.S == 0 && comp->n_rays * p.S == p.n_points && fused_composite_enabled()) {
    q.comp = *comp;
    if (composited) *composited = 1;
    if (precision == DN_PREC_F16) return paper ? launch(mlp_forward48_kernel<256, 2, 8, 0x10u, 1, 0, 0, 1>) : launch(mlp_forward48_kernel<128, 2, 4, 0u, 1, 0, 0, 1>);
    return paper ? launch(mlp_forward48_kernel<256, 1, 8, 0x10u, 1, 0, 0, 1>) : launch(mlp_forward48_kernel<128, 1, 4, 0u, 1, 0, 0, 1>);
  }
  if (shipped && fixed_ok && p.mode == 0 && std::getenv("DEXNERF_G48_NO_OVERLAP") == nullptr) {
    lds += static_cast<size_t>(kG48Waves) * 3 * kG48PointsPerWave * sizeof(float);
    if (precision == DN_PREC_F16) return launch(mlp_forward48_kernel<128, 2, 4, 0u, 1, 0, 1>);
    return launch(mlp_forward48_kernel<128, 1, 4, 0u, 1, 0, 1>);
  }
  if (paper && fixed_ok && p.mode == 0 && std::getenv("DEXNERF_G48_NO_OVERLAP") == nullptr) {
    if (precision == DN_PREC_F16) return launch(mlp_forward48_kernel<256, 2, 8, 0x10u, 1, 0, 2>);
    return launch(mlp_forward48_kernel<256, 1, 8, 0x10u, 1, 0, 2>);
  }
  if (precision == DN_PREC_F16) {
    if (paper && fixed_ok) return launch(mlp_forward48_kernel<256, 2, 8, 0x10u, 1>);
    if (shipped && fixed_ok) return launch(mlp_forward48_kernel<128, 2, 4, 0u, 1>);
    return d.hidden_size == 256 ? launch(mlp_forward48_kernel<256, 2>) : launch(mlp_forward48_kernel<128, 2>);
  }
  if (paper && fixed_ok) return launch(mlp_forward48_kernel<256, 1, 8, 0x10u, 1>);
  if (shipped && fixed_ok) return launch(mlp_forward48_kernel<128, 1, 4, 0u, 1>);
  return d.hidden_size == 256 ? launch(mlp_forward48_kernel<256, 1>) : launch(mlp_forward48_kernel<128, 1>);
}

}
```

### dex-nerf_amd/csrc/mlp_fused48_kernel.h

```cpp
#pragma once
#include "mlp_stage48.h"

namespace dn {


template <bool MAY_BE_IDENTITY = true>
__device__ __forceinline__ float pe_value(float xc, f32x4 entry) {
  const float rev = __builtin_amdgcn_fractf(xc * entry[0]) + entry[1];
  const float s = __builtin_amdgcn_sinf(rev);
  if constexpr (MAY_BE_IDENTITY) return entry[2] * xc + entry[3] * s;
  else return s;
}

__device__ __forceinline__ void rotate3(const float (&x)[3], int g, float (&xr)[3]) {
  const unsigned r = static_cast<unsigned>(g) % 3u;
  const unsigned m1 = 0u - (r & 1u), m2 = 0u - (r >> 1);
  const unsigned b0 = __float_as_uint(x[0]), b1 = __float_as_uint(x[1]), b2 = __float_as_uint(x[2]);
  xr[0] = __uint_as_float(b0 ^ ((b0 ^ b1) & m1) ^ ((b0 ^ b2) & m2));
  xr[1] = __uint_as_float(b1 ^ ((b1 ^ b2) & m1) ^ ((b1 ^ b0) & m2));
  xr[2] = __uint_as_float(b2 ^ ((b2 ^ b0) & m1) ^ ((b2 ^ b1) & m2));
}

template <int W, int F, int DC = 0, unsigned MASKC = 0, int VIEWC = 0, int SAVE = 0, int OVLP = 0, int COMP = 0>
__global__ __launch_bounds__(kG48Waves * 64, 2) void mlp_forward48_kernel(FwdParams p, G48Params q) {
  static_assert(SAVE == 0 || ((SAVE == 2 || SAVE == 3) && F == 1), "saved tensors: the 8-bit layout, bf16 arithmetic");
  static_assert(SAVE != 3 || (OVLP == 0 && COMP == 0 && DC > 0), "two point groups per wave: the fixed-shape training forward");
  static_assert(COMP == 0 || (SAVE == 0 && OVLP == 0 && DC > 0), "in-kernel compositing: a render instance whose xyz stash is free at the end of a pass");
  constexpr bool OVL = OVLP == 1;
  static_assert(!OVL || (DC >= 3 && MASKC == 0u && VIEWC != 0 && SAVE == 0 && W == 128),
                "overlapped encoding: fixed shape, no skip layer (the stash is dead after layer1), two trunk stages of 24 output tiles");
  constexpr bool OVX = OVLP == 2;
  static_assert(!OVX || (W == 256 && DC > 0 && VIEWC != 0 && SAVE == 0 && COMP == 0), "in-stage encoding: the explicit-schedule W = 256 render instance");
  constexpr int VSETS = OVL ? 3 : 2;
  constexpr int IN_ROWS = 7 + 3 * VSETS;
  constexpr bool FIXED = DC > 0;
  constexpr bool XS = FIXED && SAVE == 0 && (OVLP == 0 || OVLP == 2) && COMP == 0 && VIEWC != 0;
  constexpr bool ST = !FIXED;
  constexpr int PH = (FIXED && W == 256 && SAVE == 0) ? 2 * kPhasePieces : kPhasePieces;
  using BP8 = typename Prec<F>::BPiece;
  using Elem = typename Prec<F>::Elem;
  constexpr int PT = SAVE == 3 ? 2 : 3;
  constexpr int NT = W / 16;
  constexpr int KH = W / 32;
  constexpr int KXP = kG48XyzPieces, KDP = kG48DirPieces;
  constexpr int WAVES = kG48Waves;
  constexpr int PPW = 16 * PT;
  constexpr int PPG = kG48Waves * PPW;

  if constexpr (SAVE != 0) asm volatile("s_setreg_imm32_b32 hwreg(HW_REG_MODE, 23, 1), 1");
  extern __shared__ __attribute__((aligned(16))) char smem[];
  char* ring = smem;
  char* bias_lds = smem + kRingBytes;
  const char* tab_lds = bias_lds + q.bias_bytes;

  const int lane = threadIdx.x & 63;
  const int wave = __builtin_amdgcn_readfirstlane(threadIdx.x >> 6);
  auto fresh_lane = [&]() { int t = threadIdx.x; asm volatile("" : "+v"(t)); return t & 63; };
  auto pex_of = [&](int ln) { return smem + kRingBytes + q.bias_bytes + kG48TableBytes + wave * (PT * KXP * kPieceBytes) + ln * 16; };
  float* inbuf = reinterpret_cast<float*>(smem + kRingBytes + q.bias_bytes + kG48TableBytes + WAVES * PT * KXP * kPieceBytes) +
                 wave * (IN_ROWS * PPW);
  static_assert(OVL || IN_ROWS == kG48InRows, "g48_lds_bytes sizes the input rows");

  const int n_points = static_cast<int>(p.n_points);
  auto issue_inputs = [&](int tile, int vset) {
    const int lane = fresh_lane();
    int pt = tile * PPG + wave * PPW + lane;
    if (pt >= n_points) pt = n_points - 1;
    auto dma = [&](const float* src, int row) {
      if (lane < PPW)
        __builtin_amdgcn_global_load_lds((const __attribute__((address_space(1))) void*)src,
                                         (__attribute__((address_space(3))) void*)(inbuf + row * PPW), 4, 0, 0);
    };
    if (p.mode == 0) {
      const float* r = p.rays + static_cast<long long>(pt / p.S) * p.ray_stride;
#pragma unroll
      for (int c = 0; c < 6; ++c) dma(r + c, c);
      dma(p.z + pt, 6);
      if (p.use_viewdirs) {
#pragma unroll
        for (int c = 0; c < 3; ++c) dma(r + 8 + c, 7 + 3 * vset + c);
      }
    } else {
#pragma unroll
      for (int c = 0; c < 3; ++c) dma(p.pts + static_cast<long long>(pt) * 3 + c, c);
      if (p.use_viewdirs) {
        const float* v = p.viewdirs + static_cast<long long>(pt / p.S) * 3;
#pragma unroll
        for (int c = 0; c < 3; ++c) dma(v + c, 7 + 3 * vset + c);
      }
    }
  };

  {
    const f32x4* gsrc = reinterpret_cast<const f32x4*>(q.base);
    f32x4* l = reinterpret_cast<f32x4*>(bias_lds);
    for (int i = threadIdx.x; i < (q.bias_bytes + kG48TableBytes) / 16; i += WAVES * 64) l[i] = gsrc[i];
  }
  issue_inputs(blockIdx.x, 0);
  const unsigned inbuf_addr = static_cast<unsigned>(reinterpret_cast<uintptr_t>((__attribute__((address_space(3))) char*)inbuf));
  auto issue_inputs_flat = [&](int tile, int set) {
    const int ln = fresh_lane();
    int pt = tile * PPG + wave * PPW + ln;
    pt = pt < n_points ? pt : n_points - 1;
    const float* r = p.rays + static_cast<long long>(pt / p.S) * p.ray_stride;
#pragma unroll
    for (int c = 0; c < 6; ++c) dma4_lanes48(r + c, inbuf_addr + c * (PPW * 4));
    dma4_lanes48(p.z + pt, inbuf_addr + 6 * (PPW * 4));
#pragma unroll
    for (int c = 0; c < 3; ++c) dma4_lanes48(r + 8 + c, inbuf_addr + (7 + c) * (PPW * 4) + set * (3 * PPW * 4));
  };

  Pipe48<WAVES> pipe;
  pipe.ring = ring;
  pipe.ring_addr = static_cast<unsigned>(reinterpret_cast<uintptr_t>((__attribute__((address_space(3))) char*)ring));
  pipe.lane16 = lane * 16;
  pipe.wsrc = q.base + q.bias_bytes + kG48TableBytes;
  pipe.total_bytes = static_cast<unsigned>(q.total_pieces) * kPieceBytes;
  pipe.q_issue = 0;
  pipe.slot_wr = 0;
  pipe.wave = wave;
#pragma unroll
  for (int ph = 0; ph < (PH == kPhasePieces ? kRingPhases - 1 : kRingPhases - 2); ++ph) pipe.issue_phase();
  if constexpr (PH == kPhasePieces) {
    g48_prologue_wait(wave);
    __builtin_amdgcn_s_barrier();
  } else {
    asm volatile("s_waitcnt vmcnt(0) lgkmcnt(0)" ::: "memory");
    __syncthreads();
  }
  pipe.slot_nxt = 0;
  auto bias_at = [&](int tile) { return pipe.ring_addr + kRingBytes + ((fresh_lane() >> 4) << 4) + tile * 64; };
  pipe.rda_cur = pipe.ring_addr + lane * 16;
  pipe.slot_cur_base = pipe.ring_addr;
  static_for<PipeGeo48::PREFETCH - 1>([&](auto e_c) { pipe.template prologue_read<decltype(e_c)::value>(); });
  pipe.template bias_prefetch<0>(bias_at(0));
  pipe.template prologue_read<PipeGeo48::PREFETCH - 1>();

  unsigned trk = 0;
  int vset = 0;
  float tfreq[OVL ? 16 : 1], tphase[OVL ? 16 : 1], tw_id[3], tw_sin[3];
  float xr_n[PT][3];
  BP8 encp;
  if constexpr (OVL) {
    const f32x4* tabx = reinterpret_cast<const f32x4*>(tab_lds) + (lane >> 4) * 16;
#pragma unroll
    for (int u = 0; u < 16; ++u) {
      const f32x4 e = tabx[u];
      tfreq[u] = e[0]; tphase[u] = e[1];
      if (u < 3) { tw_id[u] = e[2]; tw_sin[u] = e[3]; }
    }
  }
  unsigned long long idm[3] = {0ull, 0ull, 0ull};
  if constexpr (OVX) {
    const f32x4* tabx = reinterpret_cast<const f32x4*>(tab_lds) + (lane >> 4) * 16;
#pragma unroll
    for (int u = 0; u < 3; ++u) idm[u] = __ballot(tabx[u][2] != 0.0f);
  }
  const int n_tiles = static_cast<int>(p.n_tiles);
  for (int tile = blockIdx.x; tile < n_tiles; tile += gridDim.x, vset = (VSETS == 2 ? vset ^ 1 : (vset == 2 ? 0 : vset + 1))) {
    const char* act_grp[PT] = {};
    const char* mask_base = nullptr;
    if constexpr (SAVE != 0) {
      const long long wt = static_cast<long long>(tile) * WAVES + wave;
#pragma unroll
      for (int t = 0; t < PT; ++t) {
        const long long G = wt * PT + t;
        act_grp[t] = uniform_ptr(p.act + ((G >> 1) * p.act_pieces * 2 + (G & 1)) * kPieceBytes);
      }
      mask_base = uniform_ptr(p.masks + wt * p.mask_words * (2 * kPieceBytes));
    }
    const bool first_tile = tile == static_cast<int>(blockIdx.x);
    if ((!OVL && !OVX) || first_tile) {
      const int ln = fresh_lane();
      const int j = ln & 15;
      const f32x4* tabx = reinterpret_cast<const f32x4*>(tab_lds) + (ln >> 4) * 16;
      char* pex = pex_of(ln);
      if (wave >= 4) asm volatile("s_waitcnt vmcnt(0)" ::: "memory");
      float in[PT][7];
#pragma unroll
      for (int t = 0; t < PT; ++t)
#pragma unroll
        for (int c = 0; c < 7; ++c) in[t][c] = inbuf[c * PPW + t * 16 + j];
      asm volatile("s_waitcnt lgkmcnt(0)" ::: "memory");
      {
        const int nxt = tile + gridDim.x;
        if (nxt < n_tiles) issue_inputs(nxt, vset ^ 1);
      }
#pragma unroll
      for (int t = 0; t < PT; ++t) {
        float x[3];
#pragma unroll
        for (int c = 0; c < 3; ++c)
          x[c] = (p.mode == 0) ? in[t][c] + in[t][3 + c] * in[t][6] : in[t][c];
        float xr[3];
        rotate3(x, ln >> 4, xr);
        BP8 pk[KXP];
#pragma unroll
        for (int k = 0; k < KXP; ++k) {
          BP8 piece;
#pragma unroll
          for (int e = 0; e < 8; ++e)
            piece[e] = static_cast<Elem>((k * 8 + e < 3) ? pe_value<true>(xr[(k * 8 + e) % 3], tabx[k * 8 + e])
                                                         : pe_value<false>(xr[(k * 8 + e) % 3], tabx[k * 8 + e]));
          *reinterpret_cast<BP8*>(pex + (t * KXP + k) * kPieceBytes) = piece;
          pk[k] = piece;
        }
        if constexpr (SAVE != 0) {
          static_assert(KXP == 2, "the xyz panel is one saved unit");
          typedef unsigned u32x4_ __attribute__((ext_vector_type(4)));
          auto cv = [](unsigned d0, unsigned d1) { return cvt_pairs_8bit<false>(d0, d1, 1.0f); };
          const u32x4_ a = __builtin_bit_cast(u32x4_, pk[0]), b = __builtin_bit_cast(u32x4_, pk[1]);
          store16_unit48(act_grp[t], static_cast<unsigned>(p.slot_xyz) * (2 * kPieceBytes), static_cast<unsigned>(ln) * 16u,
                             make_uint4(cv(a[0], a[1]), cv(a[2], a[3]), cv(b[0], b[1]), cv(b[2], b[3])));
        }
      }
    }
    auto pe_xyz = [&](int t, int k) { return *reinterpret_cast<const BP8*>(pex_of(pipe.lane16 >> 4) + (t * KXP + k) * kPieceBytes); };
    auto no_pe = [&](int, int) { return BP8{}; };
    typedef unsigned u32x4 __attribute__((ext_vector_type(4)));
    unsigned maskw[PT][2];
    auto mask_clear = [&]() {
#pragma unroll
      for (int t = 0; t < PT; ++t) { maskw[t][0] = 0u; maskw[t][1] = 0u; }
    };
    auto to_e4m3 = [](unsigned d0, unsigned d1) { return cvt_pairs_8bit<false>(d0, d1, 1.0f); };
    auto save_unit = [&](auto t_c, int slot, const BP8& lo, const BP8& hi) {
      if constexpr (SAVE != 0) {
        constexpr int t = decltype(t_c)::value;
        const u32x4 a = __builtin_bit_cast(u32x4, lo), b = __builtin_bit_cast(u32x4, hi);
        store16_unit48(act_grp[t], static_cast<unsigned>(slot) * (2 * kPieceBytes), pipe.lane16,
                           make_uint4(to_e4m3(a[0], a[1]), to_e4m3(a[2], a[3]), to_e4m3(b[0], b[1]), to_e4m3(b[2], b[3])));
      }
    };
    auto mask_tail = [&](auto nt_c, auto t_c, const auto& bo) {
      if constexpr (SAVE != 0) {
        constexpr int nt = decltype(nt_c)::value, t = decltype(t_c)::value;
        const u32x4 w = __builtin_bit_cast(u32x4, bo[nt / 2]);
        const unsigned ones = 0x00010001u;
#pragma unroll
        for (int d = 0; d < 2; ++d) {
          const unsigned pair = w[(nt & 1) * 2 + d];
          unsigned m;
          asm("v_pk_min_u16 %0, %1, %2" : "=v"(m) : "v"(pair), "s"(ones));
          unsigned mw = maskw[t][nt >> 3];
          asm volatile("v_lshl_or_b32 %0, %1, %2, %0" : "+v"(mw) : "v"(m), "n"((nt & 7) * 2 + d));
          maskw[t][nt >> 3] = mw;
        }
      }
    };
    auto unit_tail = [&](auto nt_c, auto t_c, const auto& bo, int slot0) {
      if constexpr (SAVE != 0) {
        constexpr int nt = decltype(nt_c)::value;
        if constexpr (nt % 4 == 3) save_unit(t_c, slot0 + nt / 4, bo[nt / 2 - 1], bo[nt / 2]);
      }
    };
    auto mask_store = [&](int stage) {
      if constexpr (SAVE != 0) {
        store16_uniform_at(mask_base, static_cast<unsigned>(stage) * (2 * kPieceBytes), pipe.lane16, make_uint4(maskw[0][0], maskw[0][1], maskw[1][0], maskw[1][1]));
        if constexpr (PT == 3)
          store16_uniform_at(mask_base, static_cast<unsigned>(stage) * (2 * kPieceBytes) + kPieceBytes, pipe.lane16, make_uint4(maskw[PT - 1][0], maskw[PT - 1][1], 0u, 0u));
      }
    };
    constexpr int KHU = KH / 2;

    BP8 ba[PT][KH], bb[PT][KH];
    int bias_tile = 0;
    float out4[PT][4];
    if constexpr (XS) {
      static_assert(DC >= 2 && KDP == 1, "a trunk behind layer1; the view-direction panel is one piece");
      constexpr int PX = PH;
      f32x4 pacc[PT];
      auto nothing = [&](auto) {};
      {
        BP8 pe[PT][KXP];
#pragma unroll
        for (int t = 0; t < PT; ++t)
#pragma unroll
          for (int k = 0; k < KXP; ++k) pe[t][k] = pe_xyz(t, k);
        run_stage48x<F, PX, NT, KXP, 0, 0, false, 0, 6, 0, 0>(pipe, pe, no_pe, bias_at(0), 0u, pacc,
            [&](auto nt_c, auto s_c) { hidden_op48<F, false, decltype(nt_c)::value, decltype(s_c)::value>(pacc, ba); }, nothing);
      }
      bias_tile += NT;
      static_for<DC - 1>([&](auto i_c) {
        constexpr int i = decltype(i_c)::value;
        constexpr int P0 = xs_trunk_pos(i, NT, KH, KXP, MASKC) % PX;
        auto& bin = (i % 2 == 0) ? ba : bb;
        auto& bout = (i % 2 == 0) ? bb : ba;
        auto ops = [&](auto nt_c, auto s_c) { hidden_op48<F, true, decltype(nt_c)::value, decltype(s_c)::value>(pacc, bout); };
        auto pend = [&](auto s_c) { hidden_op48<F, (i > 0), NT - 1, decltype(s_c)::value>(pacc, bin); };
        constexpr int PN = i > 0 ? 12 : 6;
        constexpr int BY = (NT - 1) / 2;
        if constexpr ((MASKC >> i) & 1u) {
          BP8 pe[PT][KXP];
#pragma unroll
          for (int t = 0; t < PT; ++t)
#pragma unroll
            for (int k = 0; k < KXP; ++k) pe[t][k] = pe_xyz(t, k);
          run_stage48x<F, PX, NT, KH, KXP, P0, false, 0, 12, PN, BY, (i == 0 ? 2 : 1)>(pipe, bin, [&](int t, int k) { return pe[t][k]; }, bias_at(bias_tile), 0u, pacc, ops, pend, &trk);
        } else {
          run_stage48x<F, PX, NT, KH, 0, P0, false, 0, 12, PN, BY, (i == 0 ? 2 : 1)>(pipe, bin, no_pe, bias_at(bias_tile), 0u, pacc, ops, pend, &trk);
        }
        bias_tile += NT;
      });
      auto& hx = ((DC - 1) % 2 == 0) ? ba : bb;
      auto& hy = ((DC - 1) % 2 == 0) ? bb : ba;
      constexpr int POS_A = xs_trunk_pos(DC - 1, NT, KH, KXP, MASKC) % PX;
      run_stage48x<F, PX, 1, KH, 0, POS_A, false, 0, 3, (DC > 1 ? 12 : 6), (NT - 1) / 2>(pipe, hx, no_pe, bias_at(bias_tile), 0u, pacc,
          [&](auto, auto s_c) { constexpr int t = decltype(s_c)::value; pick_op48(out4[t][3], pacc[t][0]); },
          [&](auto s_c) { hidden_op48<F, (DC > 1), NT - 1, decltype(s_c)::value>(pacc, hx); });
      constexpr int POS_F = (POS_A + KH) % PX;
      run_stage48x<F, PX, NT, KH, 0, POS_F, false, 0, 12, 3, KH, 1>(pipe, hx, no_pe, bias_at(bias_tile + 1), 0u, pacc,
          [&](auto nt_c, auto s_c) { hidden_op48<F, true, decltype(nt_c)::value, decltype(s_c)::value>(pacc, hy); },
          [&](auto s_c) { constexpr int t = decltype(s_c)::value; pick_op48(out4[t][3], pacc[t][0]); }, &trk);
      bias_tile += NT + 1;
      __builtin_amdgcn_sched_barrier(0);
      {
        const int ln = fresh_lane();
        const int j = ln & 15;
        const f32x4* tabd = reinterpret_cast<const f32x4*>(tab_lds + 1024) + (ln >> 4) * 8;
        char* pex = pex_of(ln);
        static_for<PT>([&](auto t_c) {
          constexpr int t = decltype(t_c)::value;
          float v[3];
#pragma unroll
          for (int c = 0; c < 3; ++c) v[c] = inbuf[(7 + 3 * vset + c) * PPW + t * 16 + j];
          float vr[3];
          rotate3(v, ln >> 4, vr);
          BP8 piece;
#pragma unroll
          for (int e = 0; e < 8; ++e) piece[e] = static_cast<Elem>((e < 3) ? pe_value<true>(vr[e % 3], tabd[e]) : pe_value<false>(vr[e % 3], tabd[e]));
          *reinterpret_cast<BP8*>(pex + t * kPieceBytes) = piece;
          __builtin_amdgcn_sched_barrier(0);
        });
      }
      __builtin_amdgcn_sched_barrier(0);
      constexpr int POS_D = (POS_F + NT * KH) % PX;
      constexpr int KT_D = KH + KDP;
      BP8 bg[PT][KH / 2];
      BP8 ped[PT];
      typedef float f32x2 __attribute__((ext_vector_type(2)));
      float ev[2] = {0.0f, 0.0f};
      f32x2 tbl[2] = {{0.0f, 0.0f}, {0.0f, 0.0f}};
      unsigned tab_addr_v = 0u, stash_addr_v = 0u;
      float in_n[PT][7];
      if constexpr (OVX) {
        static_assert(kEncOps <= enc_begin((NT / 2) * KT_D, KT_D), "the view-direction stage has a gap for every encoding op");
        {
          const unsigned must_wait = __builtin_amdgcn_readfirstlane(wave >= 4 ? 1u : 0u);
          asm volatile("s_cmp_eq_u32 %0, 0\n\t"
                       "s_cbranch_scc1 .Ldn_ovx_nowait%=\n\t"
                       "s_waitcnt vmcnt(0)\n"
                       ".Ldn_ovx_nowait%=:" ::"s"(must_wait) : "scc", "memory");
        }
        const int ln = fresh_lane();
        const int j = ln & 15;
#pragma unroll
        for (int t = 0; t < PT; ++t)
#pragma unroll
          for (int c = 0; c < 7; ++c) in_n[t][c] = inbuf[c * PPW + t * 16 + j];
        tab_addr_v = pipe.ring_addr + kRingBytes + static_cast<unsigned>(q.bias_bytes) + static_cast<unsigned>(ln >> 4) * 256u;
        stash_addr_v = pipe.ring_addr + kRingBytes + static_cast<unsigned>(q.bias_bytes) + kG48TableBytes + wave * (PT * KXP * kPieceBytes) + static_cast<unsigned>(ln) * 16u;
        asm volatile("ds_read_b64 %0, %1" : "=v"(tbl[0]) : "v"(tab_addr_v));
      }
#pragma unroll
      for (int t = 0; t < PT; ++t) ped[t] = *reinterpret_cast<const BP8*>(pex_of(pipe.lane16 >> 4) + t * kPieceBytes);
      asm volatile("s_waitcnt lgkmcnt(0)" : "+v"(ped[0]), "+v"(ped[1]), "+v"(ped[2]), "+v"(pipe.af[0]), "+v"(pipe.af[1]), "+v"(pipe.bias_nxt), "+v"(tbl[0]));
      if constexpr (OVX) {
        const int t2 = tile + 2 * static_cast<int>(gridDim.x);
        issue_inputs_flat(t2 < n_tiles ? t2 : tile, vset);
        const int ln = fresh_lane();
#pragma unroll
        for (int t = 0; t < PT; ++t) {
          float x[3];
#pragma unroll
          for (int c = 0; c < 3; ++c) x[c] = in_n[t][c] + in_n[t][3 + c] * in_n[t][6];
          rotate3(x, ln >> 4, xr_n[t]);
        }
      }
      auto enc_hook = [&](auto b_c, auto w_c) {
        if constexpr (OVX) {
          constexpr int b = decltype(b_c)::value, w = decltype(w_c)::value;
          constexpr int q0 = enc_begin(b, KT_D), cap = enc_cap(b, KT_D);
          auto one = [&](auto q_c) {
            constexpr int qq = decltype(q_c)::value;
            if constexpr (qq < kEncOps) {
              constexpr int mt = enc_table_slot_at(qq);
              constexpr int m = enc_slot_of(qq), u = m % 16, tq = m / 16, e = u % 8, k2 = u / 8;
              constexpr int kind = enc_kind(u, qq - enc_first(m));
              const unsigned ta = tab_addr_v, sa = stash_addr_v;
              if constexpr (mt >= 0) {
                f32x2& dst = tbl[mt & 1];
                asm volatile("ds_read_b64 %0, %1 offset:%2" : "=v"(dst) : "v"(ta), "n"((mt % 16) * 16));
              }
              const float xc = xr_n[tq][u % 3];
              float& val = ev[e & 1];
              const f32x2 entry = tbl[m & 1];
              if constexpr (kind == kEncMul) asm volatile("v_mul_f32 %0, %1, %2" : "=v"(val) : "v"(xc), "v"(entry[0]));
              else if constexpr (kind == kEncFract) asm volatile("v_fract_f32 %0, %0" : "+v"(val));
              else if constexpr (kind == kEncAdd) asm volatile("v_add_f32 %0, %0, %1" : "+v"(val) : "v"(entry[1]));
              else if constexpr (kind == kEncSin) asm volatile("v_sin_f32 %0, %0" : "+v"(val));
              else if constexpr (kind == kEncSel) {
                const unsigned long long im = idm[u < 3 ? u : 0];
                asm volatile("v_cndmask_b32 %0, %0, %1, %2" : "+v"(val) : "v"(xc), "s"(im));
              } else if constexpr (kind == kEncCvt) {
                typedef unsigned u32x4 __attribute__((ext_vector_type(4)));
                const float lo = ev[0], hi = ev[1];
                unsigned dw;
                if constexpr (F == 1) asm volatile("v_cvt_pk_bf16_f32 %0, %1, %2" : "=v"(dw) : "v"(lo), "v"(hi));
                else asm volatile("v_cvt_pk_f16_f32 %0, %1, %2" : "=v"(dw) : "v"(lo), "v"(hi));
                u32x4 pw = __builtin_bit_cast(u32x4, encp);
                pw[e / 2] = dw;
                encp = __builtin_bit_cast(BP8, pw);
              } else {
                const BP8 piece = encp;
                asm volatile("ds_write_b128 %0, %1 offset:%2" : : "v"(sa), "v"(piece), "n"((tq * KXP + k2) * kPieceBytes));
              }
            }
          };
          if constexpr (w < 2) one(std::integral_constant<int, q0 + w>{});
          else if constexpr (w == 2) static_for<cap - 2>([&](auto j_c) { one(std::integral_constant<int, q0 + 2 + decltype(j_c)::value>{}); });
        }
      };
      run_stage48x<F, PX, NT / 2, KH, KDP, POS_D, false, 0, 12, 12, (NT - 1) / 2, 1>(pipe, hy, [&](int t, int) { return ped[t]; }, bias_at(bias_tile), 0u, pacc,
          [&](auto nt_c, auto s_c) { hidden_op48<F, true, decltype(nt_c)::value, decltype(s_c)::value>(pacc, bg); },
          [&](auto s_c) { hidden_op48<F, true, NT - 1, decltype(s_c)::value>(pacc, hy); }, &trk, enc_hook);
      bias_tile += NT / 2;
      constexpr int POS_R = (POS_D + (NT / 2) * (KH + KDP)) % PX;
      constexpr int END = POS_R + KH / 2;
      static_assert(END <= PX && (END - 1) / kPhasePieces == POS_R / kPhasePieces, "the tail stays inside one phase");
      constexpr int PAD_R = (kPhasePieces - END % kPhasePieces) % kPhasePieces;
      static_assert((END + PAD_R) % PX == 0, "a tile pass is a whole number of barrier periods");
      run_stage48x<F, PX, 1, KH / 2, 0, POS_R, true, PAD_R, 9, 12, (NT / 2 - 1) / 2, 1>(pipe, bg, no_pe, bias_at(bias_tile), bias_at(0), pacc,
          [&](auto, auto s_c) { constexpr int sv = decltype(s_c)::value; pick_op48(out4[sv / 3][sv % 3], pacc[sv / 3][sv % 3]); },
          [&](auto s_c) { hidden_op48<F, true, NT / 2 - 1, decltype(s_c)::value>(pacc, bg); }, &trk);
      if constexpr (PAD_R != 0) pipe.template skip_xs<PX, END, PAD_R>();
      else pipe.settle();
      asm volatile("s_nop 7\n\ts_nop 1" ::: "memory");
      static_for<9>([&](auto s_c) { constexpr int sv = decltype(s_c)::value; pick_op48(out4[sv / 3][sv % 3], pacc[sv / 3][sv % 3]); });
    } else {
    {
      BP8 pe[PT][KXP];
#pragma unroll
      for (int t = 0; t < PT; ++t)
#pragma unroll
        for (int k = 0; k < KXP; ++k) pe[t][k] = pe_xyz(t, k);
      run_stage48<F, NT, KXP, 0, 0, false, ST, 0, PH>(pipe, pe, no_pe, bias_at(0), 0u, [&](auto nt_c, auto t_c, const f32x4& acc) {
        emit48<F, false, decltype(nt_c)::value>(acc, ba[decltype(t_c)::value]);
        unit_tail(nt_c, t_c, ba[decltype(t_c)::value], p.slot_layer1);
      });
    }
    bias_tile += NT;
    if constexpr (OVL) {
      {
        const unsigned must_wait = __builtin_amdgcn_readfirstlane((wave >= 4 || first_tile) ? 1u : 0u);
        asm volatile("s_cmp_eq_u32 %0, 0\n\t"
                     "s_cbranch_scc1 .Ldn_ovl_nowait%=\n\t"
                     "s_waitcnt vmcnt(0)\n"
                     ".Ldn_ovl_nowait%=:" ::"s"(must_wait) : "scc", "memory");
      }
      const int ln = fresh_lane();
      const int j = ln & 15;
      float in[PT][7];
#pragma unroll
      for (int t = 0; t < PT; ++t)
#pragma unroll
        for (int c = 0; c < 7; ++c) in[t][c] = inbuf[c * PPW + t * 16 + j];
      asm volatile("s_waitcnt lgkmcnt(0)" ::: "memory");
      {
        const int t2 = tile + 2 * static_cast<int>(gridDim.x);
        issue_inputs_flat(t2 < n_tiles ? t2 : tile, vset == 0 ? 2 : vset - 1);
      }
#pragma unroll
      for (int t = 0; t < PT; ++t) {
        float x[3];
#pragma unroll
        for (int c = 0; c < 3; ++c) x[c] = in[t][c] + in[t][3 + c] * in[t][6];
        rotate3(x, ln >> 4, xr_n[t]);
      }
    }
    auto enc_step = [&](auto m_c) {
      if constexpr (OVL) {
        constexpr int m = decltype(m_c)::value;
        constexpr int tq = m / 16, k = (m % 16) / 8, e = m % 8, u = k * 8 + e;
        static_assert(KXP == 2 && PT == 3, "48 slots per lane");
        const float xc = xr_n[tq][u % 3];
        const float rev = __builtin_amdgcn_fractf(xc * tfreq[u]) + tphase[u];
        const float sv = __builtin_amdgcn_sinf(rev);
        float val = sv;
        if constexpr (u < 3) val = tw_id[u] * xc + tw_sin[u] * sv;
        encp[e] = static_cast<Elem>(val);
        if constexpr (e == 7) *reinterpret_cast<BP8*>(pex_of(fresh_lane()) + (tq * KXP + k) * kPieceBytes) = encp;
      }
    };
    auto heads = [&](const BP8 (&hx)[PT][KH], BP8 (&hy)[PT][KH], auto view_c) __attribute__((always_inline)) {
      if constexpr (decltype(view_c)::value) {
        run_stage48<F, 1, KH, 0, 0, false, ST, 0, PH>(pipe, hx, no_pe, bias_at(bias_tile), 0u, [&](auto, auto t_c, const f32x4& acc) {
          out4[decltype(t_c)::value][3] = acc[0];
        });
        mask_clear();
        run_stage48<F, NT, KH, 0, KH % PH, false, ST, 0, PH, 1>(pipe, hx, no_pe, bias_at(bias_tile + 1), 0u, [&](auto nt_c, auto t_c, const f32x4& acc) {
          emit48<F, true, decltype(nt_c)::value>(acc, hy[decltype(t_c)::value]);
          mask_tail(nt_c, t_c, hy[decltype(t_c)::value]);
          unit_tail(nt_c, t_c, hy[decltype(t_c)::value], p.slot_feat);
        }, &trk);
        mask_store(p.D - 1);
        bias_tile += NT + 1;
        __builtin_amdgcn_sched_barrier(0);
        BP8 ped_now[PT];
        {
          const int ln = fresh_lane();
          const int j = ln & 15;
          const f32x4* tabd = reinterpret_cast<const f32x4*>(tab_lds + 1024) + (ln >> 4) * 8;
          char* pex = pex_of(ln);
          static_for<PT>([&](auto t_c) {
            constexpr int t = decltype(t_c)::value;
            float v[3];
#pragma unroll
            for (int c = 0; c < 3; ++c) v[c] = inbuf[(7 + 3 * vset + c) * PPW + t * 16 + j];
            float vr[3];
            rotate3(v, ln >> 4, vr);
            BP8 piece;
#pragma unroll
            for (int e = 0; e < 8; ++e) piece[e] = static_cast<Elem>((e < 3) ? pe_value<true>(vr[e % 3], tabd[e]) : pe_value<false>(vr[e % 3], tabd[e]));
            if constexpr (OVL) ped_now[t] = piece;
            else *reinterpret_cast<BP8*>(pex + t * kPieceBytes) = piece;
            if constexpr (SAVE != 0) {
              const u32x4 a = __builtin_bit_cast(u32x4, piece);
              const unsigned w0 = to_e4m3(a[0], a[1]), w1 = to_e4m3(a[2], a[3]);
              const auto s0 = __builtin_amdgcn_permlane32_swap(w0, w0, false, false);
              const auto s1 = __builtin_amdgcn_permlane32_swap(w1, w1, false, false);
              store16_unit48(act_grp[t], static_cast<unsigned>(p.slot_dir) * (2 * kPieceBytes), static_cast<unsigned>(ln) * 16u, make_uint4(w0, w1, s0[1], s1[1]));
            }
            __builtin_amdgcn_sched_barrier(0);
          });
        }
        __builtin_amdgcn_sched_barrier(0);
        constexpr int POS_D = ((NT + 1) * KH) % PH;
        BP8 bg[PT][KH / 2];
        BP8 ped[PT];
#pragma unroll
        for (int t = 0; t < PT; ++t) {
          if constexpr (OVL) ped[t] = ped_now[t];
          else ped[t] = *reinterpret_cast<const BP8*>(pex_of(pipe.lane16 >> 4) + t * kPieceBytes);
        }
        auto pe_dir = [&](int t, int) { return ped[t]; };
        mask_clear();
        run_stage48<F, NT / 2, KH, KDP, POS_D, false, ST, 0, PH, 1>(pipe, hy, pe_dir, bias_at(bias_tile), 0u, [&](auto nt_c, auto t_c, const f32x4& acc) {
          emit48<F, true, decltype(nt_c)::value>(acc, bg[decltype(t_c)::value]);
          mask_tail(nt_c, t_c, bg[decltype(t_c)::value]);
          unit_tail(nt_c, t_c, bg[decltype(t_c)::value], p.slot_dirout);
        }, &trk);
        mask_store(p.D);
        bias_tile += NT / 2;
        constexpr int POS_R = (POS_D + (NT / 2) * (KH + KDP)) % PH;
        constexpr int END = POS_R + KH / 2;
        static_assert(END <= PH && (END - 1) / kPhasePieces == POS_R / kPhasePieces, "the tail stays inside one phase");
        constexpr int PAD_R = (kPhasePieces - END % kPhasePieces) % kPhasePieces;
        static_assert((END + PAD_R) % PH == 0, "a tile pass is a whole number of barrier periods");
        run_stage48<F, 1, KH / 2, 0, POS_R, true, ST, PAD_R, PH, 1>(pipe, bg, no_pe, bias_at(bias_tile), bias_at(0), [&](auto, auto t_c, const f32x4& acc) {
          constexpr int t = decltype(t_c)::value;
          out4[t][0] = acc[0]; out4[t][1] = acc[1]; out4[t][2] = acc[2];
        }, &trk);
        if constexpr (PAD_R != 0) pipe.template skip<END, PAD_R, PH>();
        else pipe.settle();
      } else {
        static_assert(PH == kPhasePieces, "no-viewdirs nets run the every-phase barrier");
        run_stage48<F, 1, KH, 0, 0, true, ST, (kPhasePieces - KH % kPhasePieces) % kPhasePieces, kPhasePieces, 1>(pipe, hx, no_pe, bias_at(bias_tile), bias_at(0), [&](auto, auto t_c, const f32x4& acc) {
          constexpr int t = decltype(t_c)::value;
          out4[t][0] = acc[0]; out4[t][1] = acc[1]; out4[t][2] = acc[2]; out4[t][3] = acc[3];
        }, &trk);
        if constexpr (KH % kPhasePieces != 0) pipe.template skip<KH % kPhasePieces, kPhasePieces - KH % kPhasePieces>();
        else pipe.settle();
      }
    };
    if constexpr (FIXED) {
      static_assert((NT * KXP) % PH == 0 && (NT * KH) % PH == 0 && (NT * (KH + KXP)) % PH == 0,
                    "layer1 and every trunk layer span whole barrier periods: each stage starts at position 0 of one");
      static_for<DC - 1>([&](auto i_c) {
        constexpr int i = decltype(i_c)::value;
        auto& bin = (i % 2 == 0) ? ba : bb;
        auto& bout = (i % 2 == 0) ? bb : ba;
        auto emit = [&](auto nt_c, auto t_c, const f32x4& acc) {
          emit48<F, true, decltype(nt_c)::value>(acc, bout[decltype(t_c)::value]);
          mask_tail(nt_c, t_c, bout[decltype(t_c)::value]);
          unit_tail(nt_c, t_c, bout[decltype(t_c)::value], p.slot_trunk0 + i * KHU);
          if constexpr (OVL && i < 2) {
            static_assert(!OVL || NT * PT == 24, "two trunk stages = the 48 encoding slots of a lane");
            enc_step(std::integral_constant<int, i * 24 + decltype(nt_c)::value * PT + decltype(t_c)::value>{});
          }
        };
        mask_clear();
        if constexpr ((MASKC >> i) & 1u) {
          BP8 pe[PT][KXP];
#pragma unroll
          for (int t = 0; t < PT; ++t)
#pragma unroll
            for (int k = 0; k < KXP; ++k) pe[t][k] = pe_xyz(t, k);
          run_stage48<F, NT, KH, KXP, 0, false, false, 0, PH, (i == 0 ? 2 : 1)>(pipe, bin, [&](int t, int k) { return pe[t][k]; }, bias_at(bias_tile), 0u, emit, &trk);
        } else {
          run_stage48<F, NT, KH, 0, 0, false, false, 0, PH, (i == 0 ? 2 : 1)>(pipe, bin, no_pe, bias_at(bias_tile), 0u, emit, &trk);
        }
        mask_store(i);
        bias_tile += NT;
      });
      if constexpr ((DC - 1) % 2 == 0) heads(ba, bb, std::integral_constant<bool, VIEWC != 0>{});
      else heads(bb, ba, std::integral_constant<bool, VIEWC != 0>{});
    } else {
      auto trunk_layer = [&](int i, const BP8 (&bin)[PT][KH], BP8 (&bout)[PT][KH]) __attribute__((always_inline)) {
        auto emit = [&](auto nt_c, auto t_c, const f32x4& acc) {
          emit48<F, true, decltype(nt_c)::value>(acc, bout[decltype(t_c)::value]);
          mask_tail(nt_c, t_c, bout[decltype(t_c)::value]);
          unit_tail(nt_c, t_c, bout[decltype(t_c)::value], p.slot_trunk0 + i * KHU);
        };
        mask_clear();
        constexpr int TRK_RT = W == 128 ? 2 : 0;
        if ((p.skip_mask >> i) & 1u) run_stage48<F, NT, KH, KXP, 0, false, true, 0, kPhasePieces, TRK_RT>(pipe, bin, pe_xyz, bias_at(bias_tile), 0u, emit, &trk);
        else run_stage48<F, NT, KH, 0, 0, false, true, 0, kPhasePieces, TRK_RT>(pipe, bin, no_pe, bias_at(bias_tile), 0u, emit, &trk);
        mask_store(i);
        bias_tile += NT;
      };
      int i = 0;
      for (; i + 1 < p.D - 1; i += 2) {
        trunk_layer(i, ba, bb);
        trunk_layer(i + 1, bb, ba);
      }
      if (i < p.D - 1) {
        trunk_layer(i, ba, bb);
#pragma unroll
        for (int t = 0; t < PT; ++t)
#pragma unroll
          for (int k = 0; k < KH; ++k) ba[t][k] = bb[t][k];
      }
      if (p.use_viewdirs) heads(ba, bb, std::true_type{});
      else heads(ba, bb, std::false_type{});
    }
    }
    const int lo = fresh_lane();
    if constexpr (COMP != 0) {
      f32x4* stage = reinterpret_cast<f32x4*>(smem + kRingBytes + q.bias_bytes + kG48TableBytes);
#pragma unroll
      for (int t = 0; t < PT; ++t) {
        if (lo < 16) {
          f32x4 o;
          o[0] = out4[t][0]; o[1] = out4[t][1]; o[2] = out4[t][2]; o[3] = out4[t][3];
          stage[wave * PPW + t * 16 + lo] = o;
        }
      }
      asm volatile("s_waitcnt lgkmcnt(0)" ::: "memory");
      __builtin_amdgcn_s_barrier();
      const int S = p.S;
      const int rays_per_tile = PPG / S;
      for (int r = wave; r < rays_per_tile; r += WAVES) {
        const long long ray = static_cast<long long>(tile) * rays_per_tile + r;
        if (ray < q.comp.n_rays) {
          const f32x4* rows = stage + r * S;
          composite_ray([&](int sc) { const f32x4 r = rows[sc]; return make_float4(r[0], r[1], r[2], r[3]); }, p.z + ray * S,
                        p.rays + ray * p.ray_stride + 3, ray, lo, static_cast<const float*>(nullptr), 0.0f, q.comp.white, q.comp.th,
                        q.comp.n_thres, q.comp.n_rays, S, q.comp.rgb, q.comp.disp, q.comp.acc, q.comp.weights, q.comp.depth, q.comp.dex,
                        q.comp.nonfinite, RngRef{nullptr, 0u});
        }
      }
      asm volatile("s_waitcnt lgkmcnt(0)" ::: "memory");
      __builtin_amdgcn_s_barrier();
    } else {
#pragma unroll
      for (int t = 0; t < PT; ++t) {
        const int pt = tile * PPG + wave * PPW + t * 16 + (lo & 15);
        if (pt < n_points && lo < 16) {
          f32x4 o;
          o[0] = out4[t][0]; o[1] = out4[t][1]; o[2] = out4[t][2]; o[3] = out4[t][3];
          __builtin_nontemporal_store(o, reinterpret_cast<f32x4*>(p.out + static_cast<long long>(pt) * 4));
        }
      }
    }
  }
  asm volatile("s_waitcnt vmcnt(0) lgkmcnt(0)" ::: "memory");
  if constexpr (F == 2) {
    const bool out_of_range = (trk & 0xFFFFu) >= 0x7C00u || (trk >> 16) >= 0x7C00u;
    if (p.range_flag != nullptr && __ballot(out_of_range) != 0ull && (threadIdx.x & 63) == 0) atomicAdd(p.range_flag, 1u);
  }
}

#define DN_FWD48_PAPER_BF16(X)  \
  X(256, 1, 8, 0x10u, 1, 0, 2, 0) X(256, 1, 8, 0x10u, 1, 0, 0, 0)
#define DN_FWD48_PAPER_FP16(X)  \
  X(256, 2, 8, 0x10u, 1, 0, 2, 0) X(256, 2, 8, 0x10u, 1, 0, 0, 0)
#define DN_FWD48_W128(X)  \
  X(128, 1, 0, 0u, 0, 0, 0, 0) X(128, 2, 0, 0u, 0, 0, 0, 0)  \
  X(128, 1, 4, 0u, 1, 0, 0, 0) X(128, 2, 4, 0u, 1, 0, 0, 0)  \
  X(128, 1, 4, 0u, 1, 0, 1, 0) X(128, 2, 4, 0u, 1, 0, 1, 0)  \
  X(128, 1, 4, 0u, 1, 0, 0, 1) X(128, 2, 4, 0u, 1, 0, 0, 1)  \
  X(128, 1, 4, 0u, 1, 2, 0, 0) X(128, 1, 4, 0u, 1, 3, 0, 0) X(128, 1, 0, 0u, 0, 2, 0, 0)
#define DN_FWD48_HOST_UNIT(X)  \
  X(256, 1, 0, 0u, 0, 0, 0, 0) X(256, 2, 0, 0u, 0, 0, 0, 0)        \
  X(256, 1, 8, 0x10u, 1, 0, 0, 1) X(256, 2, 8, 0x10u, 1, 0, 0, 1)  \
  X(256, 1, 8, 0x10u, 1, 2, 0, 0) X(256, 1, 8, 0x10u, 1, 3, 0, 0) X(256, 1, 0, 0u, 0, 2, 0, 0)
#define DN_FWD48_INSTANCES(X) DN_FWD48_PAPER_BF16(X) DN_FWD48_PAPER_FP16(X) DN_FWD48_W128(X) DN_FWD48_HOST_UNIT(X)

#define DN_FWD48_INSTANTIATE(W, F, DC, MASKC, VIEWC, SAVE, OVLP, COMP) \
  template __global__ void mlp_forward48_kernel<W, F, DC, MASKC, VIEWC, SAVE, OVLP, COMP>(FwdParams, G48Params);
#define DN_FWD48_EXTERN(W, F, DC, MASKC, VIEWC, SAVE, OVLP, COMP) extern DN_FWD48_INSTANTIATE(W, F, DC, MASKC, VIEWC, SAVE, OVLP, COMP)

}
```

### dex-nerf_amd/csrc/mlp_geo48.h

```cpp
#pragma once
#include "mlp_internal.h"
#include "composite_body.h"

namespace dn {

constexpr int kG48Waves = 8;
constexpr int kG48PointsPerWave = 48;
constexpr int kG48PointsPerWg = kG48Waves * kG48PointsPerWave;
constexpr int kG48XyzPieces = kXyzPanel / 32;
constexpr int kG48DirPieces = 1;
constexpr int kG48TableBytes = 1536;
constexpr int kG48InRows = 13;

__host__ __device__ inline int g48_pe_col(int kind, int g, int u, int L) {
  const int slots = kind == 1 ? 16 : 8;
  const int comp = (u + g) % 3;
  int rank = 0;
  for (int gg = 0; gg <= g; ++gg)
    for (int uu = 0; uu < (gg == g ? u : slots); ++uu) rank += ((uu + gg) % 3 == comp) ? 1 : 0;
  if (rank == 0) return comp;
  const int f = (rank - 1) / 2, is_cos = (rank - 1) % 2;
  return f < L ? 3 + 6 * f + 3 * is_cos + comp : -1;
}

__host__ __device__ constexpr int g48_hidden_col(int k, int g, int e) { return (2 * k + e / 4) * 16 + 4 * g + (e % 4); }

struct G48Tables {
  float fx[16];
  float fd[8];
  int LX, LD;
};

struct G48Params {
  const char* base;
  int bias_bytes;
  int total_pieces;
  CompParams comp;
};


inline int build_layout48(const dn_mlp_desc& d, NetLayout* out) {
  const int W = d.hidden_size, D = d.num_layers;
  const int DX = 3 + 6 * d.num_encoding_fn_xyz, DD = 3 + 6 * d.num_encoding_fn_dir;
  NetLayout& L = *out;
  L = NetLayout{};
  L.W = W; L.LX = d.num_encoding_fn_xyz; L.LD = d.num_encoding_fn_dir; L.D = D; L.use_viewdirs = d.use_viewdirs;
  int piece = 0, bias = 0, s = 0;
  auto add = [&](int n_tiles, int hidden_in, int pe_kind, int src, int src2, int n_real, int ld, int col_h0, int col_p0) {
    StageDesc& t = L.st[s++];
    t = StageDesc{};
    t.n_tiles = n_tiles; t.hidden_in = hidden_in; t.pe_kind = pe_kind; t.src = src; t.src2 = src2;
    t.n_real = n_real; t.ld = ld; t.col_hidden0 = col_h0; t.col_pe0 = col_p0;
    t.first_tile2 = (src2 >= 0) ? 0 : -1;
    t.pieces_per_tile = hidden_in / 32 + (pe_kind == 1 ? kG48XyzPieces : (pe_kind == 2 ? kG48DirPieces : 0));
    t.piece0 = piece; t.bias0 = bias;
    piece += n_tiles * t.pieces_per_tile;
    bias += n_tiles;
  };
  const int NT = W / 16;
  add(NT, 0, 1, 0, -1, W, DX, 0, 0);
  for (int i = 0; i < D - 1; ++i) {
    const bool wide = (i % d.skip_connect_every == 0) && i > 0 && i != D - 1;
    if (wide) L.skip_mask |= (1u << i);
    add(NT, W, wide ? 1 : 0, 1 + i, -1, W, wide ? W + DX : W, 0, W);
  }
  if (d.use_viewdirs) {
    const int i_dir = D, i_alpha = D + 1, i_rgb = D + 2, i_feat = D + 3;
    add(NT + 1, W, 0, i_feat, i_alpha, W, W, 0, 0);
    add(NT / 2, W, 2, i_dir, -1, W / 2, W + DD, 0, W);
    add(1, W / 2, 0, i_rgb, -1, 3, W / 2, 0, 0);
  } else {
    add(1, W, 0, D, -1, 4, W, 0, 0);
  }
  L.n_stages = s;
  L.total_pieces = round_up(piece, kPhasePieces);
  L.total_bias_tiles = bias;
  L.bias_bytes = round_up(bias * 64, 1024);
  return 0;
}

inline size_t g48_lds_bytes(const NetLayout& L) {
  return static_cast<size_t>(kRingBytes) + L.bias_bytes + kG48TableBytes + kG48Waves * 3 * kG48XyzPieces * kPieceBytes +
         kG48Waves * kG48InRows * kG48PointsPerWave * sizeof(float);
}

inline bool g48_supported(const dn_mlp_desc& d, int precision) {
  if ((precision != DN_PREC_BF16 && precision != DN_PREC_F16) || (d.hidden_size != 256 && d.hidden_size != 128)) return false;
  NetLayout L;
  build_layout48(d, &L);
  return g48_lds_bytes(L) <= 160 * 1024;
}

inline unsigned pack48_blocks(const NetLayout& L) {
  const long long elems = static_cast<long long>(L.total_pieces) * 512;
  const long long b = (elems + 511) / 512;
  return static_cast<unsigned>(b < 64 ? 64 : (b > 4096 ? 4096 : b));
}

inline size_t g48_region_bytes(const dn_mlp_desc& d) {
  NetLayout L;
  build_layout48(d, &L);
  return static_cast<size_t>(L.bias_bytes) + kG48TableBytes + static_cast<size_t>(L.total_pieces) * kPieceBytes;
}

bool g48_range_guard_complete(const dn_mlp_desc& d);
constexpr int kS8BlockBytes = 256;
enum { kS8BlockSaturated = 0, kS8BlockFloor = 1, kS8BlockSampled = 2,
       kS8BlockScale = 4,
       kS8BlockStats = 8,
       kS8BlockReplicas = 8,
       kS8BlockPartials = 40,
       kS8BlockPartialCount = 24 };

struct TrainLayout48 {
  int32_t kh_u;
  int32_t act_units;
  int32_t slot_xyz, slot_dir, slot_layer1, slot_trunk0, slot_feat, slot_dirout;
  int32_t mask_stages;
  int32_t grad_units;
  int32_t gslot_dirout, gslot_feat, gslot_trunk0, gslot_layer1;
  int32_t gslot_out;
};

inline void build_train_layout48(const dn_mlp_desc& d, TrainLayout48* t) {
  const int W = d.hidden_size, D = d.num_layers;
  t->kh_u = W / 64;
  int s = 0;
  t->slot_xyz = s; s += 1;
  t->slot_dir = s; s += d.use_viewdirs ? 1 : 0;
  t->slot_layer1 = s; s += t->kh_u;
  t->slot_trunk0 = s; s += (D - 1) * t->kh_u;
  t->slot_feat = s; s += d.use_viewdirs ? t->kh_u : 0;
  t->slot_dirout = s; s += d.use_viewdirs ? W / 128 : 0;
  t->act_units = s;
  t->mask_stages = (D - 1) + (d.use_viewdirs ? 2 : 0);
  int g = 0;
  t->gslot_dirout = g; g += d.use_viewdirs ? W / 128 : 0;
  t->gslot_feat = g; g += d.use_viewdirs ? t->kh_u : 0;
  t->gslot_trunk0 = g; g += (D - 1) * t->kh_u;
  t->gslot_layer1 = g; g += t->kh_u;
  t->gslot_out = g; g += 1;
  t->grad_units = g;
}

inline long long g48_padded_records(long long n_points) {
  const long long r3 = (n_points + 383) / 384 * 12, r2 = (n_points + 255) / 256 * 8;
  return r3 > r2 ? r3 : r2;
}
inline long long g48_mask_wave_tiles(long long n_points) {
  return (n_points + 255) / 256 * kG48Waves;
}
inline bool g48_two_group_shape(const dn_mlp_desc& d) {
  NetLayout L;
  build_layout48(d, &L);
  const bool paper = d.hidden_size == 256 && d.num_layers == 8 && L.skip_mask == 0x10u && d.use_viewdirs;
  const bool shipped = d.hidden_size == 128 && d.num_layers == 4 && L.skip_mask == 0u && d.use_viewdirs;
  return (paper || shipped) && std::getenv("DEXNERF_G48_RUNTIME_SHAPE") == nullptr;
}
inline int g48_train_groups(long long n_points, int cus) {
  if (const char* e = std::getenv("DEXNERF_G48_TRAIN_GROUPS")) {
    const int v = std::atoi(e);
    if (v == 2 || v == 3) return v;
  }
  if (cus < 1) cus = 1;
  const long long t3 = (n_points + 383) / 384, t2 = (n_points + 255) / 256;
  const long long c3 = (t3 + cus - 1) / cus * 3, c2 = (t2 + cus - 1) / cus * 2;
  return c2 * 100 <= c3 * 75 ? 2 : 3;
}

inline bool g48_train_supported(const dn_mlp_desc& d) {
  return g48_supported(d, DN_PREC_BF16) && train_lxyz_supported(d);
}

inline int build_backward_layout48(const dn_mlp_desc& d, NetLayout* out) {
  const int W = d.hidden_size, D = d.num_layers;
  const int DX = 3 + 6 * d.num_encoding_fn_xyz, DD = 3 + 6 * d.num_encoding_fn_dir;
  NetLayout& L = *out;
  L = NetLayout{};
  L.W = W; L.LX = d.num_encoding_fn_xyz; L.LD = d.num_encoding_fn_dir; L.D = D; L.use_viewdirs = d.use_viewdirs;
  int piece = 0, s = 0;
  auto add = [&](int n_rows, int k_hidden, int custom, int src, int src2, int ld) {
    StageDesc& t = L.st[s++];
    t = StageDesc{};
    t.n_tiles = n_rows / 16; t.hidden_in = k_hidden; t.src = src; t.src2 = src2;
    t.n_real = n_rows; t.ld = ld; t.first_tile2 = -1; t.transposed = 1; t.custom_k = custom;
    t.pieces_per_tile = k_hidden / 32 + (custom > 0 ? 1 : 0);
    t.piece0 = piece;
    piece += t.n_tiles * t.pieces_per_tile;
  };
  for (int i = 0; i < D - 1; ++i)
    if ((i % d.skip_connect_every == 0) && i > 0 && i != D - 1) L.skip_mask |= (1u << i);
  if (d.use_viewdirs) {
    const int i_dir = D, i_alpha = D + 1, i_rgb = D + 2, i_feat = D + 3;
    add(W / 2, 0, 3, i_rgb, -1, W / 2);
    add(W, W / 2, 0, i_dir, -1, W + DD);
    add(W, W, 1, i_feat, i_alpha, W);
  } else {
    add(W, 0, 4, D, -1, W);
  }
  for (int i = D - 2; i >= 0; --i) {
    const bool wide = (L.skip_mask >> i) & 1u;
    add(W, W, 0, 1 + i, -1, wide ? W + DX : W);
  }
  L.n_stages = s;
  L.total_pieces = round_up(piece, kPhasePieces);
  return 0;
}

int launch_pack48(const dn_mlp_desc& d, int precision, const PackPtrs& ptrs, char* region, hipStream_t stream);
int launch_forward48(const dn_mlp_desc& d, int precision, const FwdParams& p, const char* region, hipStream_t stream,
                     const CompParams* comp = nullptr, int* composited = nullptr);
int backward48_entry(const dn_mlp_desc* desc, const void* packed_bwd, const float* g_out, const void* masks, int64_t n_points,
                     void* grads, float grad_scale, hipStream_t stream, const unsigned* partials = nullptr, int n_partials = 0);
int unpack48_entry(const dn_mlp_desc* desc, int which, const void* native, int64_t n_points, int slot, int width, int kind, float* out,
                   int ld_out, int col0, hipStream_t stream);
int launch_pack48_pair(const dn_mlp_desc& d, const PackPtrs& a, const PackPtrs& b, char* region_a, char* region_b, hipStream_t stream);
int launch_pack48_backward_pair(const dn_mlp_desc& d, const PackPtrs& a, const PackPtrs& b, char* packed_a, char* packed_b, hipStream_t stream);
int launch_pack48_backward(const dn_mlp_desc& d, const PackPtrs& ptrs, char* packed, hipStream_t stream);

}
```

### dex-nerf_amd/csrc/mlp_internal.h

```cpp
#pragma once
#include "mlp_device.h"

namespace dn {

struct PackPtrs {
  const float* w[kMaxStages];
  const float* b[kMaxStages];
};

int setup_params(const dn_mlp_desc* desc, int precision, const void* packed, FwdParams* p);
struct CompParams;
int dispatch_forward(const dn_mlp_desc& d, int precision, FwdParams& p, hipStream_t stream, const CompParams* comp = nullptr, int* composited = nullptr);
int launch_pack(const NetLayout& L, const PackPtrs& ptrs, void* packed, int precision, hipStream_t stream);

}
```

### dex-nerf_amd/csrc/mlp_stage48.h

```cpp
#pragma once
#include <type_traits>
#include "mlp_geo48.h"

namespace dn {

using PipeGeo48 = PipeGeometry<true, true, true, 2>;
template <int WAVES>
using Pipe48 = PipeT<WAVES, PipeGeo48>;

__device__ __forceinline__ void g48_prologue_wait(unsigned wave) {
  const unsigned fetcher = __builtin_amdgcn_readfirstlane(wave < 4 ? 1u : 0u);
  asm volatile("s_cmp_eq_u32 %0, 0\n\t"
               "s_cbranch_scc1 .Ldn_prol_all%=\n\t"
               "s_waitcnt vmcnt(8) lgkmcnt(0)\n\t"
               "s_branch .Ldn_prol_done%=\n"
               ".Ldn_prol_all%=:\n\t"
               "s_waitcnt vmcnt(0) lgkmcnt(0)\n"
               ".Ldn_prol_done%=:" ::"s"(fetcher) : "scc", "memory");
}

template <int F>
__device__ __forceinline__ f32x4 mfma48(typename Prec<F>::BPiece a, typename Prec<F>::BPiece b, f32x4 c) {
  if constexpr (F == 1) return __builtin_amdgcn_mfma_f32_16x16x32_bf16(a, b, c, 0, 0, 0);
  else return __builtin_amdgcn_mfma_f32_16x16x32_f16(a, b, c, 0, 0, 0);
}

template <bool LAST, int END, int PAD>
constexpr int g48_issued(int q0, int q1) {
  int n = 0;
  for (int q = q0; q < q1; ++q) n += (LAST && q >= END && q < END + PAD) ? 0 : 1;
  return n;
}

template <int F, int NT_OUT, int KH, int KP, int POS0, bool LAST = false, bool SETTLE = true, int PAD = 0, int PH = kPhasePieces, int TRK = 0,
          bool BIAS = true, class PipeT, class BH, class BP, class Emit>
__device__ __forceinline__ void run_stage48(PipeT& pipe, const BH& bh, BP&& bp, unsigned bias_addr, unsigned next_addr, Emit&& emit,
                                            unsigned* trk = nullptr) {
  constexpr int PT = static_cast<int>(std::extent<BH, 0>::value), KT = KH + KP;
  static_assert(PT == 2 || PT == 3, "bh is [point groups][pieces]");
  static_assert(KT >= 2 || !BIAS, "the bias prefetch distance assumes at least two pieces per tile");
  static_for<NT_OUT>([&](auto nt_c) {
    constexpr int nt = decltype(nt_c)::value;
    f32x4 acc[PT];
    static_for<KT>([&](auto k_c) {
      constexpr int k = decltype(k_c)::value;
      constexpr int pos = POS0 + nt * KT + k;
      pipe.template at_position<PH, pos>();
      if constexpr (k == 0) {
        f32x4 b = {0.0f, 0.0f, 0.0f, 0.0f};
        if constexpr (BIAS) b = pipe.template bias_take<1>();
#pragma unroll
        for (int t = 0; t < PT; ++t) acc[t] = b;
      }
      constexpr int newer = g48_issued<LAST, POS0 + NT_OUT * KT, PAD>(pos + 1, pos + PipeGeo48::PREFETCH) + ((BIAS && k == KT - 1) ? 1 : 0);
      const auto a = __builtin_bit_cast(typename Prec<F>::BPiece, pipe.template take<pos, newer>());
      static_for<PT>([&](auto t_c) {
        constexpr int t = decltype(t_c)::value;
        if constexpr (k < KH) acc[t] = mfma48<F>(a, bh[t][k], acc[t]);
        else acc[t] = mfma48<F>(a, bp(t, k - KH), acc[t]);
      });
      if constexpr (g48_issued<LAST, POS0 + NT_OUT * KT, PAD>(pos + PipeGeo48::PREFETCH, pos + PipeGeo48::PREFETCH + 1) == 1) pipe.template prefetch<pos>();
      if constexpr (BIAS && k == KT - 2) {
        if constexpr (nt + 1 < NT_OUT) pipe.template bias_prefetch<(nt + 1) * 64>(bias_addr);
        else if constexpr (LAST) pipe.template bias_prefetch<0>(next_addr);
        else pipe.template bias_prefetch<NT_OUT * 64>(bias_addr);
      }
    });
    __builtin_amdgcn_sched_barrier(0);
    static_for<PT>([&](auto t_c) { emit(nt_c, t_c, acc[decltype(t_c)::value]); });
    if constexpr (F == 2 && TRK != 0) {
      typedef unsigned u32x4 __attribute__((ext_vector_type(4)));
      constexpr int TOT = PT * KH * 4;
      constexpr int Q0 = nt * TOT / NT_OUT, Q1 = (nt + 1) * TOT / NT_OUT;
      auto dword = [&](int q) { return __builtin_bit_cast(u32x4, bh[q / (KH * 4)][(q / 4) % KH])[q % 4]; };
      if constexpr (TRK == 2) {
        static_for<Q1 - Q0>([&](auto q_c) {
          const unsigned v = dword(Q0 + decltype(q_c)::value);
          unsigned t = *trk;
          unsigned tmp;
          asm volatile("v_and_b32 %1, 0x7fff7fff, %2\n\tv_pk_max_u16 %0, %0, %1" : "+v"(t), "=&v"(tmp) : "v"(v));
          *trk = t;
        });
      } else {
        static_for<(Q1 - Q0 + 1) / 2>([&](auto q_c) {
          constexpr int qa = Q0 + 2 * decltype(q_c)::value, qb = (qa + 1 < Q1) ? qa + 1 : qa;
          const unsigned va = dword(qa), vb = dword(qb);
          unsigned t = *trk;
          asm volatile("v_pk_maximum3_f16 %0, %0, %1, %2" : "+v"(t) : "v"(va), "v"(vb));
          *trk = t;
        });
      }
    }
  });
  if constexpr (SETTLE) pipe.template settle<BIAS>();
}

template <int F>
__device__ __forceinline__ void mfma48_first(f32x4& d, const f32x4& a, const typename Prec<F>::BPiece& b, const f32x4& c) {
  if constexpr (F == 1) asm volatile("v_mfma_f32_16x16x32_bf16 %0, %1, %2, %3" : "=&v"(d) : "v"(a), "v"(b), "v"(c));
  else asm volatile("v_mfma_f32_16x16x32_f16 %0, %1, %2, %3" : "=&v"(d) : "v"(a), "v"(b), "v"(c));
}
#define DN_XS_WAIT "s_waitcnt lgkmcnt(%[n])\n\t"
template <int F, int NEWER>
__device__ __forceinline__ void mfma48_first_w(f32x4& d, f32x4& a, const typename Prec<F>::BPiece& b, const f32x4& c) {
  if constexpr (F == 1) asm volatile(DN_XS_WAIT "v_mfma_f32_16x16x32_bf16 %[d], %[a], %[b], %[c]" : [d] "=&v"(d), [a] "+v"(a) : [b] "v"(b), [c] "v"(c), [n] "n"(NEWER));
  else asm volatile(DN_XS_WAIT "v_mfma_f32_16x16x32_f16 %[d], %[a], %[b], %[c]" : [d] "=&v"(d), [a] "+v"(a) : [b] "v"(b), [c] "v"(c), [n] "n"(NEWER));
}
template <int F, int NEWER>
__device__ __forceinline__ void mfma48_acc_w(f32x4& d, f32x4& a, const typename Prec<F>::BPiece& b) {
  if constexpr (F == 1) asm volatile(DN_XS_WAIT "v_mfma_f32_16x16x32_bf16 %[d], %[a], %[b], %[d]" : [d] "+v"(d), [a] "+v"(a) : [b] "v"(b), [n] "n"(NEWER));
  else asm volatile(DN_XS_WAIT "v_mfma_f32_16x16x32_f16 %[d], %[a], %[b], %[d]" : [d] "+v"(d), [a] "+v"(a) : [b] "v"(b), [n] "n"(NEWER));
}
template <int F>
__device__ __forceinline__ void mfma48_acc(f32x4& d, const f32x4& a, const typename Prec<F>::BPiece& b) {
  if constexpr (F == 1) asm volatile("v_mfma_f32_16x16x32_bf16 %0, %1, %2, %0" : "+v"(d) : "v"(a), "v"(b));
  else asm volatile("v_mfma_f32_16x16x32_f16 %0, %1, %2, %0" : "+v"(d) : "v"(a), "v"(b));
}

template <int F, bool RELU, int NT, int S, class BSet>
__device__ __forceinline__ void hidden_op48(const f32x4 (&pacc)[3], BSet& bo) {
  typedef unsigned u32x4 __attribute__((ext_vector_type(4)));
  static_assert(S >= 0 && S < (RELU ? 12 : 6), "op index");
  constexpr int t = (S % 6) / 2, d = S % 2, e = (NT & 1) * 2 + d;
  u32x4 w = __builtin_bit_cast(u32x4, bo[t][NT / 2]);
  if constexpr (S < 6) {
    const float x = pacc[t][2 * d], y = pacc[t][2 * d + 1];
    unsigned o;
    if constexpr (F == 1) asm volatile("v_cvt_pk_bf16_f32 %0, %1, %2" : "=v"(o) : "v"(x), "v"(y));
    else asm volatile("v_cvt_pk_f16_f32 %0, %1, %2" : "=v"(o) : "v"(x), "v"(y));
    w[e] = o;
  } else {
    unsigned o = w[e];
    asm volatile("v_pk_max_i16 %0, %0, 0" : "+v"(o));
    w[e] = o;
  }
  bo[t][NT / 2] = __builtin_bit_cast(typename Prec<F>::BPiece, w);
}
__device__ __forceinline__ void pick_op48(float& dst, float src) { asm volatile("v_mov_b32 %0, %1" : "=v"(dst) : "v"(src)); }

constexpr int xs_blocks(int np, int kt, int deadline) {
  int e = kt < 6 ? kt : 6;
  if (deadline < e) e = deadline;
  if (e < 1) e = 1;
  (void)np;
  return e;
}
constexpr int xs_per(int np, int e) { return (np + e - 1) / e; }
constexpr int xs_trunk_pos(int i, int nt, int kh, int kxp, unsigned mask) {
  int p = nt * kxp;
  for (int j = 0; j < i; ++j) p += nt * (kh + (((mask >> j) & 1u) ? kxp : 0));
  return p;
}

constexpr int enc_slot_len(int u) { return 4 + (u < 3 ? 1 : 0) + ((u % 8) % 2) + ((u % 8) == 7 ? 1 : 0); }
constexpr int enc_first(int m) {
  int q = 0;
  for (int i = 0; i < m; ++i) q += enc_slot_len(i % 16);
  return q;
}
constexpr int kEncSlots = 48;
constexpr int kEncOps = enc_first(kEncSlots);
constexpr int enc_slot_of(int q) {
  int m = 0;
  while (m < kEncSlots && q >= enc_slot_len(m % 16)) { q -= enc_slot_len(m % 16); ++m; }
  return m;
}
enum { kEncMul = 0, kEncFract = 1, kEncAdd = 2, kEncSin = 3, kEncSel = 4, kEncCvt = 5, kEncWrite = 6 };
constexpr int enc_kind(int u, int idx) {
  if (idx < 4) return idx;
  int j = 4;
  if (u < 3) { if (idx == j) return kEncSel; ++j; }
  if ((u % 8) % 2) { if (idx == j) return kEncCvt; ++j; }
  return kEncWrite;
}
constexpr int enc_cap(int b, int kt) { return (b % kt) >= 6 ? 4 : 3; }
constexpr int enc_begin(int b, int kt) {
  int q = 0;
  for (int i = 0; i < b; ++i) q += enc_cap(i, kt);
  return q;
}
constexpr int kEncLead = 5;
constexpr int enc_table_slot_at(int q) {
  for (int m = 1; m < kEncSlots; ++m)
    if (enc_first(m) - kEncLead == q) return m;
  return -1;
}

struct XsNoHook {
  template <class B, class W>
  __device__ __forceinline__ void operator()(B, W) const {}
};
template <int F, int PX, int NT_OUT, int KH, int KP, int POS0, bool LAST, int PAD, int NOPS, int PEND_N, int PEND_BY, int TRK = 0, class PipeT, class BH,
          class BP, class Ops, class Pend, class Hook = XsNoHook>
__device__ __forceinline__ void run_stage48x(PipeT& pipe, const BH& bh, BP&& bp, unsigned bias_addr, unsigned next_addr, f32x4 (&pacc)[3],
                                             Ops&& ops, Pend&& pend, unsigned* trk = nullptr, Hook&& hook = Hook{}) {
  constexpr int PT = 3, KT = KH + KP;
  static_assert(KT >= 2 && KH >= 1, "the bias prefetch distance assumes at least two pieces per tile; a tile's first piece is a hidden piece");
  static_for<NT_OUT>([&](auto nt_c) {
    constexpr int nt = decltype(nt_c)::value;
    constexpr int NP = nt == 0 ? PEND_N : NOPS;
    constexpr int E = xs_blocks(NP, KT, nt == 0 ? PEND_BY : KT);
    constexpr int PER = xs_per(NP, E);
    static_assert(PER * E >= NP, "every pending op has a slot");
    constexpr int TOT = (F == 2 && TRK != 0) ? PT * KH * 4 : 0;
    constexpr int Q0 = nt * TOT / NT_OUT, Q1 = (nt + 1) * TOT / NT_OUT;
    constexpr int NTRK = (TRK == 2) ? (Q1 - Q0) : (Q1 - Q0 + 1) / 2;
    constexpr int TB = KT - E > 0 ? KT - E : 1;
    constexpr int TPER = (NTRK + TB - 1) / TB;
    auto run_op = [&](auto s_c) {
      constexpr int sidx = decltype(s_c)::value;
      if constexpr (sidx < NP) {
        if constexpr (nt == 0) pend(s_c);
        else ops(std::integral_constant<int, nt - 1>{}, s_c);
      }
    };
    auto run_trk = [&](auto q_c) {
      constexpr int qi = decltype(q_c)::value;
      if constexpr (qi < NTRK) {
        typedef unsigned u32x4 __attribute__((ext_vector_type(4)));
        auto dword = [&](int q) { return __builtin_bit_cast(u32x4, bh[q / (KH * 4)][(q / 4) % KH])[q % 4]; };
        unsigned tv = *trk;
        if constexpr (TRK == 2) {
          const unsigned v = dword(Q0 + qi);
          unsigned tmp;
          asm volatile("v_and_b32 %1, 0x7fff7fff, %2\n\tv_pk_max_u16 %0, %0, %1" : "+v"(tv), "=&v"(tmp) : "v"(v));
        } else {
          constexpr int qa = Q0 + 2 * qi, qb = (qa + 1 < Q1) ? qa + 1 : qa;
          const unsigned va = dword(qa), vb = dword(qb);
          asm volatile("v_pk_maximum3_f16 %0, %0, %1, %2" : "+v"(tv) : "v"(va), "v"(vb));
        }
        *trk = tv;
      }
    };
    f32x4 acc[PT];
    static_for<KT>([&](auto k_c) {
      constexpr int k = decltype(k_c)::value;
      constexpr int pos = POS0 + nt * KT + k;
      pipe.template at_position_xs<PX, pos>();
      f32x4 b = {0.0f, 0.0f, 0.0f, 0.0f};
      if constexpr (k == 0) b = pipe.template bias_take<1>();
      constexpr int newer = g48_issued<LAST, POS0 + NT_OUT * KT, PAD>(pos + 1, pos + PipeGeo48::PREFETCH) + ((k == KT - 1) ? 1 : 0);
      f32x4& a = pipe.af[pos % PipeGeo48::PREFETCH];
      static_for<PT>([&](auto t_c) {
        constexpr int t = decltype(t_c)::value;
        if constexpr (t == 0) {
          if constexpr (k == 0) mfma48_first_w<F, newer>(acc[t], a, bh[t][0], b);
          else if constexpr (k < KH) mfma48_acc_w<F, newer>(acc[t], a, bh[t][k]);
          else mfma48_acc_w<F, newer>(acc[t], a, bp(t, k - KH));
        } else if constexpr (k == 0) mfma48_first<F>(acc[t], a, bh[t][0], b);
        else if constexpr (k < KH) mfma48_acc<F>(acc[t], a, bh[t][k]);
        else mfma48_acc<F>(acc[t], a, bp(t, k - KH));
        if constexpr (k < E) {
          if constexpr (t < 2) run_op(std::integral_constant<int, k * PER + t>{});
          else static_for<(PER > 2 ? PER - 2 : 0)>([&](auto j_c) { run_op(std::integral_constant<int, k * PER + 2 + decltype(j_c)::value>{}); });
        } else if constexpr (NTRK > 0) {
          constexpr int kb = (KT - E > 0) ? k - E : 0;
          if constexpr (t < 2) run_trk(std::integral_constant<int, kb * TPER + t>{});
          else static_for<(TPER > 2 ? TPER - 2 : 0)>([&](auto j_c) { run_trk(std::integral_constant<int, kb * TPER + 2 + decltype(j_c)::value>{}); });
        }
        hook(std::integral_constant<int, nt * KT + k>{}, t_c);
      });
      if constexpr (KT - E <= 0 && NTRK > 0 && k == KT - 1)
        static_for<NTRK>([&](auto q_c) { run_trk(q_c); });
      pipe.template xs_after_piece<PX, pos>();
      hook(std::integral_constant<int, nt * KT + k>{}, std::integral_constant<int, 3>{});
      if constexpr (g48_issued<LAST, POS0 + NT_OUT * KT, PAD>(pos + PipeGeo48::PREFETCH, pos + PipeGeo48::PREFETCH + 1) == 1) pipe.template prefetch<pos>();
      if constexpr (k == KT - 2) {
        if constexpr (nt + 1 < NT_OUT) pipe.template bias_prefetch<(nt + 1) * 64>(bias_addr);
        else if constexpr (LAST) pipe.template bias_prefetch<0>(next_addr);
        else pipe.template bias_prefetch<NT_OUT * 64>(bias_addr);
      }
    });
#pragma unroll
    for (int t = 0; t < PT; ++t) pacc[t] = acc[t];
  });
}

template <int F, bool RELU, int NT, class BO>
__device__ __forceinline__ void emit48(const f32x4& acc, BO& bo) {
  typedef float f32x2 __attribute__((ext_vector_type(2)));
  typedef typename Prec<F>::Elem e16x2 __attribute__((ext_vector_type(2)));
  typedef short s16x2 __attribute__((ext_vector_type(2)));
  typedef unsigned u32x4 __attribute__((ext_vector_type(4)));
  u32x4 w = __builtin_bit_cast(u32x4, bo[NT / 2]);
#pragma unroll
  for (int d = 0; d < 2; ++d) {
    f32x2 f = {acc[2 * d], acc[2 * d + 1]};
    e16x2 v = __builtin_convertvector(f, e16x2);
    if constexpr (RELU) {
      s16x2 bits = __builtin_bit_cast(s16x2, v);
      const s16x2 zero = {0, 0};
      bits = __builtin_elementwise_max(bits, zero);
      v = __builtin_bit_cast(e16x2, bits);
    }
    w[(NT & 1) * 2 + d] = __builtin_bit_cast(unsigned, v);
  }
  bo[NT / 2] = __builtin_bit_cast(typename Prec<F>::BPiece, w);
}

}
```

Before: 5.279 million rays/s.

## Skip the view-direction stage for wavefront tiles whose density is all zero

Adds a transparent-tile skip to the bf16 48-geometry forward kernel. While the feature layer runs, each wave ORs an LDS verdict word that records whether any of its points has positive sigma. Tiles whose points are all non-positive skip the feature tail and the view-direction/RGB stages, zero their colour outputs, and resynchronise the weight-streaming ring. It also adds 'pinning' asm constraints so the ring bookkeeping stays in scalar registers. The change adds LDS traffic, a barrier and a data-dependent branch, and it only helps when many tiles are empty space.

```diff
diff --git a/dex-nerf_amd/csrc/api.cpp b/dex-nerf_amd/csrc/api.cpp
--- a/dex-nerf_amd/csrc/api.cpp
+++ b/dex-nerf_amd/csrc/api.cpp
@@ -87,6 +87,11 @@
   return carve(nullptr, n_rays, num_coarse, num_fine).bytes;
 }
 
+static bool tile_skip_enabled() {
+  const char* e = std::getenv("DEXNERF_TILE_SKIP");
+  return e == nullptr || std::atoi(e) != 0;
+}
+
 extern "C" int dn_render_rays(const dn_mlp_desc* desc_coarse, const void* packed_coarse, const dn_mlp_desc* desc_fine,
                               const void* packed_fine, int precision, const float* rays, int ray_stride,
                               int64_t n_rays, int num_coarse, int num_fine, int lindisp, float noise_std,
@@ -116,11 +121,12 @@
     return c;
   };
   const bool may_fuse = !(noise_std > 0.0f);
+  const int skip = (may_fuse && precision == DN_PREC_BF16 && tile_skip_enabled()) ? 1 : 0;
   int done = 0;
   {
     const CompParams c = comp_for(rgb_c, acc_c, w.w_c, depth_c, fine ? nullptr : dex_f, fine ? 0 : n_thres);
     if ((rc = run_network_flagged(desc_coarse, precision, packed_coarse, nullptr, nullptr, rays, ray_stride, w.z_c, n_rays,
-                                  num_coarse, w.rf_c, w.status + 1, stream, (may_fuse && rgb_c) ? &c : nullptr, &done)))
+                                  num_coarse, w.rf_c, w.status + 1, stream, (may_fuse && rgb_c) ? &c : nullptr, &done, skip)))
       return rc;
   }
   if (!done && (rc = volume_render_counting(w.rf_c, w.z_c, rays + 3, ray_stride, noise_c, noise_std, white_background, h_m_thres,
@@ -132,7 +138,7 @@
   {
     const CompParams c = comp_for(rgb_f, acc_f, nullptr, depth_f, dex_f, n_thres);
     if ((rc = run_network_flagged(desc_fine, precision, packed_fine, nullptr, nullptr, rays, ray_stride, w.z_f, n_rays,
-                                  num_coarse + num_fine, w.rf_f, w.status + 1, stream, (may_fuse && rgb_f) ? &c : nullptr, &done)))
+                                  num_coarse + num_fine, w.rf_f, w.status + 1, stream, (may_fuse && rgb_f) ? &c : nullptr, &done, skip)))
       return rc;
   }
   if (done) return 0;
diff --git a/dex-nerf_amd/csrc/dn_common.h b/dex-nerf_amd/csrc/dn_common.h
--- a/dex-nerf_amd/csrc/dn_common.h
+++ b/dex-nerf_amd/csrc/dn_common.h
@@ -35,7 +35,8 @@
 struct CompParams;
 int run_network_flagged(const dn_mlp_desc* desc, int precision, const void* packed, const float* pts, const float* viewdirs,
                         const float* rays, int ray_stride, const float* z_vals, int64_t n_rays, int samples_per_ray, float* out,
-                        unsigned* range_flag, dn_stream_t stream, const CompParams* comp = nullptr, int* composited = nullptr);
+                        unsigned* range_flag, dn_stream_t stream, const CompParams* comp = nullptr, int* composited = nullptr,
+                        int skip_transparent = 0);
 
 int coarse_depths_rng(const float* rays, int ray_stride, int64_t n_rays, int num_coarse, int lindisp, const float* t_rand,
                       float* z_vals, const uint32_t* rng_state, dn_stream_t stream);
diff --git a/dex-nerf_amd/csrc/mlp_device.h b/dex-nerf_amd/csrc/mlp_device.h
--- a/dex-nerf_amd/csrc/mlp_device.h
+++ b/dex-nerf_amd/csrc/mlp_device.h
@@ -221,7 +221,7 @@
   }
   unsigned long long xs_src[2];
   unsigned xs_dst[2];
-  template <int PERIOD>
+  template <int PERIOD, bool PIN = false>
   __device__ __forceinline__ void xs_period_begin() {
     static_assert(PERIOD == kPhasePieces || PERIOD == 2 * kPhasePieces, "barrier period: one or two phases");
     if constexpr (PERIOD == 2 * kPhasePieces) asm volatile("s_waitcnt vmcnt(0)" ::: "memory");
@@ -235,6 +235,10 @@
       const unsigned hi = __builtin_amdgcn_readfirstlane(static_cast<unsigned>(bits >> 32));
       xs_src[h] = (static_cast<unsigned long long>(hi) << 32) | lo;
       xs_dst[h] = __builtin_amdgcn_readfirstlane(ring_addr + pend_dst);
+    }
+    if constexpr (PIN) {
+      static_assert(PERIOD == 2 * kPhasePieces, "pinned bookkeeping: the two-phase period");
+      asm volatile("" : "+s"(xs_src[0]), "+s"(xs_src[1]), "+s"(xs_dst[0]), "+s"(xs_dst[1]), "+s"(q_issue), "+s"(slot_wr));
     }
   }
   template <int PERIOD, int Q>
@@ -257,13 +261,14 @@
         : [wave] "s"(wave), [who] "n"(Q / STEPS), [lds] "s"(xs_dst[H]), [voff] "v"(lane16), [sbase] "s"(xs_src[H]), [o0] "n"(OFF), [o1] "n"(OFF + 1024)
         : "memory", "scc");
   }
-  template <int PERIOD, int POS>
+  template <int PERIOD, int POS, bool PIN = false>
   __device__ __forceinline__ void at_position_xs() {
-    if constexpr (POS % PERIOD == 0) xs_period_begin<PERIOD>();
+    if constexpr (POS % PERIOD == 0) xs_period_begin<PERIOD, PIN>();
     if constexpr (POS % kPhasePieces == 0) {
       slot_nxt = (slot_nxt + 1 == kRingPhases) ? 0 : slot_nxt + 1;
       rda_cur = slot_cur_base + lane16;
       slot_cur_base = __builtin_amdgcn_readfirstlane(ring_addr + slot_nxt * kSlotBytes);
+      if constexpr (PIN) asm volatile("" : "+s"(slot_nxt), "+s"(slot_cur_base));
     }
   }
   template <int PERIOD, int POS>
diff --git a/dex-nerf_amd/csrc/mlp_fused.hip b/dex-nerf_amd/csrc/mlp_fused.hip
--- a/dex-nerf_amd/csrc/mlp_fused.hip
+++ b/dex-nerf_amd/csrc/mlp_fused.hip
@@ -109,13 +109,15 @@
   return check_launch("mlp_forward");
 }
 
-int dispatch_forward(const dn_mlp_desc& d, int precision, FwdParams& p, hipStream_t stream, const CompParams* comp, int* composited) {
+int dispatch_forward(const dn_mlp_desc& d, int precision, FwdParams& p, hipStream_t stream, const CompParams* comp, int* composited,
+                     int skip_transparent) {
   const bool bf = precision == DN_PREC_BF16;
   const bool hf = precision == DN_PREC_F16;
   const char* geom_env = getenv("DEXNERF_BF16_GEOM");
   const bool geom48 = !(geom_env && atoi(geom_env) == 32);
   if ((bf || hf) && geom48 && p.act == nullptr && p.mode != 2 && p.n_points < (1LL << 31) - 1024 && g48_supported(d, precision))
-    return launch_forward48(d, precision, p, p.packed + p.bias_bytes + static_cast<size_t>(p.total_pieces) * kPieceBytes, stream, comp, composited);
+    return launch_forward48(d, precision, p, p.packed + p.bias_bytes + static_cast<size_t>(p.total_pieces) * kPieceBytes, stream, comp, composited,
+                            skip_transparent);
   if (p.act != nullptr && hf) { set_error("mlp_forward(train): fp16 is a render-only mode"); return DN_E_UNSUPPORTED; }
   if (p.act != nullptr && p.save8) {
     if (!bf || p.mode == 2 || !g48_train_supported(d) || p.n_points >= (1LL << 31) - 1024) {
@@ -227,7 +229,7 @@
 int dn::run_network_flagged(const dn_mlp_desc* desc, int precision, const void* packed, const float* pts,
                             const float* viewdirs, const float* rays, int ray_stride, const float* z_vals,
                             int64_t n_rays, int samples_per_ray, float* out, unsigned* range_flag, dn_stream_t stream,
-                            const CompParams* comp, int* composited) {
+                            const CompParams* comp, int* composited, int skip_transparent) {
   if (composited) *composited = 0;
   FwdParams p;
   int rc = setup_params(desc, precision, packed, &p);
@@ -248,7 +250,7 @@
   p.out = out;
   p.range_flag = range_flag;
   if (p.n_points == 0) return 0;
-  return dispatch_forward(*desc, precision, p, as_stream(stream), comp, composited);
+  return dispatch_forward(*desc, precision, p, as_stream(stream), comp, composited, skip_transparent);
 }
 
 extern "C" int dn_mlp_forward_encoded(const dn_mlp_desc* desc, int precision, const void* packed, const float* x,
diff --git a/dex-nerf_amd/csrc/mlp_fused48.hip b/dex-nerf_amd/csrc/mlp_fused48.hip
--- a/dex-nerf_amd/csrc/mlp_fused48.hip
+++ b/dex-nerf_amd/csrc/mlp_fused48.hip
@@ -138,13 +138,14 @@
 }
 
 int launch_forward48(const dn_mlp_desc& d, int precision, const FwdParams& p_in, const char* region, hipStream_t stream,
-                     const CompParams* comp, int* composited) {
+                     const CompParams* comp, int* composited, int skip_transparent) {
   if (composited) *composited = 0;
   NetLayout L;
   build_layout48(d, &L);
   FwdParams p = p_in;
   G48Params q{};
   q.base = region; q.bias_bytes = L.bias_bytes; q.total_pieces = L.total_pieces;
+  q.skip_transparent = (skip_transparent != 0 && precision == DN_PREC_BF16 && g48_verdict_words_fit(L)) ? 1 : 0;
   p.n_tiles = (p.n_points + kG48PointsPerWg - 1) / kG48PointsPerWg;
   size_t lds = g48_lds_bytes(L);
   if (lds > 160 * 1024) { set_error("mlp_forward48: %zu bytes of LDS", lds); return DN_E_UNSUPPORTED; }
diff --git a/dex-nerf_amd/csrc/mlp_fused48_kernel.h b/dex-nerf_amd/csrc/mlp_fused48_kernel.h
--- a/dex-nerf_amd/csrc/mlp_fused48_kernel.h
+++ b/dex-nerf_amd/csrc/mlp_fused48_kernel.h
@@ -128,6 +128,18 @@
     asm volatile("s_waitcnt vmcnt(0) lgkmcnt(0)" ::: "memory");
     __syncthreads();
   }
+  constexpr bool TSKIP = XS && F == 1 && W == 256;
+  static_assert(!(TSKIP && COMP != 0), "G48Params: skip_transparent and comp share one slot - no instance may read both");
+  constexpr int kVerdictOff = g48_paper_bias_tiles(W, DC > 0 ? DC : 1) * 64;
+  if constexpr (TSKIP) {
+    static_assert(kVerdictOff % 1024 != 0 && 1024 - kVerdictOff % 1024 >= 8, "the bias rows' padding holds the two verdict words");
+    if (threadIdx.x < 2) reinterpret_cast<unsigned*>(bias_lds + kVerdictOff)[threadIdx.x] = 0u;
+  }
+  unsigned skip_on = 0u;
+  if constexpr (TSKIP) {
+    skip_on = static_cast<unsigned>(q.skip_transparent);
+    asm volatile("" : "+s"(skip_on));
+  }
   pipe.slot_nxt = 0;
   auto bias_at = [&](int tile) { return pipe.ring_addr + kRingBytes + ((fresh_lane() >> 4) << 4) + tile * 64; };
   pipe.rda_cur = pipe.ring_addr + lane * 16;
@@ -289,6 +301,7 @@
         auto ops = [&](auto nt_c, auto s_c) { hidden_op48<F, true, decltype(nt_c)::value, decltype(s_c)::value>(pacc, bout); };
         auto pend = [&](auto s_c) { hidden_op48<F, (i > 0), NT - 1, decltype(s_c)::value>(pacc, bin); };
         constexpr int PN = i > 0 ? 12 : 6;
+        constexpr bool PIN_I = TSKIP && i == DC - 2;
         constexpr int BY = (NT - 1) / 2;
         if constexpr ((MASKC >> i) & 1u) {
           BP8 pe[PT][KXP];
@@ -296,9 +309,9 @@
           for (int t = 0; t < PT; ++t)
 #pragma unroll
             for (int k = 0; k < KXP; ++k) pe[t][k] = pe_xyz(t, k);
-          run_stage48x<F, PX, NT, KH, KXP, P0, false, 0, 12, PN, BY, (i == 0 ? 2 : 1)>(pipe, bin, [&](int t, int k) { return pe[t][k]; }, bias_at(bias_tile), 0u, pacc, ops, pend, &trk);
+          run_stage48x<F, PX, NT, KH, KXP, P0, false, 0, 12, PN, BY, (i == 0 ? 2 : 1), PIN_I>(pipe, bin, [&](int t, int k) { return pe[t][k]; }, bias_at(bias_tile), 0u, pacc, ops, pend, &trk);
         } else {
-          run_stage48x<F, PX, NT, KH, 0, P0, false, 0, 12, PN, BY, (i == 0 ? 2 : 1)>(pipe, bin, no_pe, bias_at(bias_tile), 0u, pacc, ops, pend, &trk);
+          run_stage48x<F, PX, NT, KH, 0, P0, false, 0, 12, PN, BY, (i == 0 ? 2 : 1), PIN_I>(pipe, bin, no_pe, bias_at(bias_tile), 0u, pacc, ops, pend, &trk);
         }
         bias_tile += NT;
       });
@@ -309,9 +322,141 @@
           [&](auto, auto s_c) { constexpr int t = decltype(s_c)::value; pick_op48(out4[t][3], pacc[t][0]); },
           [&](auto s_c) { hidden_op48<F, (DC > 1), NT - 1, decltype(s_c)::value>(pacc, hx); });
       constexpr int POS_F = (POS_A + KH) % PX;
-      run_stage48x<F, PX, NT, KH, 0, POS_F, false, 0, 12, 3, KH, 1>(pipe, hx, no_pe, bias_at(bias_tile + 1), 0u, pacc,
-          [&](auto nt_c, auto s_c) { hidden_op48<F, true, decltype(nt_c)::value, decltype(s_c)::value>(pacc, hy); },
-          [&](auto s_c) { constexpr int t = decltype(s_c)::value; pick_op48(out4[t][3], pacc[t][0]); }, &trk);
+      auto sigma_pend = [&](auto s_c) { constexpr int t = decltype(s_c)::value; pick_op48(out4[t][3], pacc[t][0]); };
+      constexpr int NT_A = (PX - POS_F) / KH;
+      bool transparent = false;
+      if constexpr (TSKIP) {
+        static_assert(PX == 2 * kPhasePieces, "the transparent path's ring accounting is the two-phase period's");
+        static_assert((POS_F + NT_A * KH) % PX == 0 && NT_A >= 1 && NT_A + 1 < NT, "fc_feat's tile NT_A opens a barrier period");
+        const unsigned vw_addr = pipe.ring_addr + kRingBytes + kVerdictOff;
+        unsigned verdict = 0u;
+        run_stage48x<F, PX, NT_A, KH, 0, POS_F, false, 0, 12, 3, KH, 1>(pipe, hx, no_pe, bias_at(bias_tile + 1), 0u, pacc,
+            [&](auto nt_c, auto s_c) { hidden_op48<F, true, decltype(nt_c)::value, decltype(s_c)::value>(pacc, hy); }, sigma_pend, &trk,
+            [&](auto b_c, auto w_c) {
+              if constexpr (decltype(b_c)::value == 3 && decltype(w_c)::value == 3) {
+                const bool lv = fresh_lane() < 16 && (!(out4[0][3] <= 0.0f) || !(out4[1][3] <= 0.0f) || !(out4[2][3] <= 0.0f));
+                const unsigned flag = __ballot(lv) != 0ull ? 1u : 0u;
+                const unsigned a = vw_addr + static_cast<unsigned>(vset) * 4u;
+                asm volatile("ds_or_b32 %0, %1" : : "v"(a), "v"(flag));
+              }
+            });
+        run_stage48x<F, PX, 1, KH, 0, (POS_F + NT_A * KH) % PX, false, 0, 12, 12, KH, 1>(pipe, hx, no_pe, bias_at(bias_tile + 1 + NT_A), 0u, pacc,
+            [&](auto, auto s_c) { hidden_op48<F, true, NT_A, decltype(s_c)::value>(pacc, hy); },
+            [&](auto s_c) { hidden_op48<F, true, NT_A - 1, decltype(s_c)::value>(pacc, hy); }, &trk,
+            [&](auto b_c, auto w_c) {
+              if constexpr (decltype(b_c)::value == 0 && decltype(w_c)::value == 3) {
+                const unsigned a = vw_addr + static_cast<unsigned>(vset) * 4u, o = vw_addr + static_cast<unsigned>(vset ^ 1) * 4u, zero = 0u;
+                unsigned& dst = verdict;
+                asm volatile("ds_read_b32 %0, %1" : "=v"(dst) : "v"(a));
+                asm volatile("ds_write_b32 %0, %1" : : "v"(o), "v"(zero));
+              }
+            });
+        pipe.settle();
+        transparent = skip_on != 0u && __builtin_amdgcn_readfirstlane(verdict) == 0u;
+      }
+      BP8 bg[PT][KH / 2];
+      BP8 ped[PT];
+      typedef float f32x2 __attribute__((ext_vector_type(2)));
+      float ev[2] = {0.0f, 0.0f};
+      f32x2 tbl[2] = {{0.0f, 0.0f}, {0.0f, 0.0f}};
+      unsigned tab_addr_v = 0u, stash_addr_v = 0u;
+      float in_n[PT][7];
+      auto enc_one = [&](auto q_c) {
+        constexpr int qq = decltype(q_c)::value;
+        if constexpr (OVX && qq < kEncOps) {
+          constexpr int mt = enc_table_slot_at(qq);
+          constexpr int m = enc_slot_of(qq), u = m % 16, tq = m / 16, e = u % 8, k2 = u / 8;
+          constexpr int kind = enc_kind(u, qq - enc_first(m));
+          const unsigned ta = tab_addr_v, sa = stash_addr_v;
+          if constexpr (mt >= 0) {
+            f32x2& dst = tbl[mt & 1];
+            asm volatile("ds_read_b64 %0, %1 offset:%2" : "=v"(dst) : "v"(ta), "n"((mt % 16) * 16));
+          }
+          const float xc = xr_n[tq][u % 3];
+          float& val = ev[e & 1];
+          const f32x2 entry = tbl[m & 1];
+          if constexpr (kind == kEncMul) asm volatile("v_mul_f32 %0, %1, %2" : "=v"(val) : "v"(xc), "v"(entry[0]));
+          else if constexpr (kind == kEncFract) asm volatile("v_fract_f32 %0, %0" : "+v"(val));
+          else if constexpr (kind == kEncAdd) asm volatile("v_add_f32 %0, %0, %1" : "+v"(val) : "v"(entry[1]));
+          else if constexpr (kind == kEncSin) asm volatile("v_sin_f32 %0, %0" : "+v"(val));
+          else if constexpr (kind == kEncSel) {
+            const unsigned long long im = idm[u < 3 ? u : 0];
+            asm volatile("v_cndmask_b32 %0, %0, %1, %2" : "+v"(val) : "v"(xc), "s"(im));
+          } else if constexpr (kind == kEncCvt) {
+            typedef unsigned u32x4 __attribute__((ext_vector_type(4)));
+            const float lo = ev[0], hi = ev[1];
+            unsigned dw;
+            if constexpr (F == 1) asm volatile("v_cvt_pk_bf16_f32 %0, %1, %2" : "=v"(dw) : "v"(lo), "v"(hi));
+            else asm volatile("v_cvt_pk_f16_f32 %0, %1, %2" : "=v"(dw) : "v"(lo), "v"(hi));
+            u32x4 pw = __builtin_bit_cast(u32x4, encp);
+            pw[e / 2] = dw;
+            encp = __builtin_bit_cast(BP8, pw);
+          } else {
+            const BP8 piece = encp;
+            asm volatile("ds_write_b128 %0, %1 offset:%2" : : "v"(sa), "v"(piece), "n"((tq * KXP + k2) * kPieceBytes));
+          }
+        }
+      };
+      if (TSKIP && transparent) {
+        if constexpr (TSKIP) {
+          asm volatile("s_waitcnt vmcnt(0)" ::: "memory");
+          __builtin_amdgcn_s_barrier();
+          const unsigned s0 = pipe.slot_wr;
+          pipe.q_issue = 0;
+          pipe.issue_phase();
+          pipe.issue_phase();
+          pipe.issue_phase();
+          pipe.slot_nxt = s0;
+          pipe.slot_cur_base = __builtin_amdgcn_readfirstlane(pipe.ring_addr + s0 * kSlotBytes);
+          if constexpr (OVX) {
+            const int ln = fresh_lane();
+            const int j = ln & 15;
+#pragma unroll
+            for (int t = 0; t < PT; ++t)
+#pragma unroll
+              for (int c = 0; c < 7; ++c) in_n[t][c] = inbuf[c * PPW + t * 16 + j];
+            tab_addr_v = pipe.ring_addr + kRingBytes + static_cast<unsigned>(q.bias_bytes) + static_cast<unsigned>(ln >> 4) * 256u;
+            stash_addr_v = pipe.ring_addr + kRingBytes + static_cast<unsigned>(q.bias_bytes) + kG48TableBytes + wave * (PT * KXP * kPieceBytes) + static_cast<unsigned>(ln) * 16u;
+            asm volatile("ds_read_b64 %0, %1" : "=v"(tbl[0]) : "v"(tab_addr_v));
+            asm volatile("s_waitcnt lgkmcnt(0)" : "+v"(tbl[0]) : : "memory");
+            const int t2 = tile + 2 * static_cast<int>(gridDim.x);
+            issue_inputs_flat(t2 < n_tiles ? t2 : tile, vset);
+#pragma unroll
+            for (int t = 0; t < PT; ++t) {
+              float x[3];
+#pragma unroll
+              for (int c = 0; c < 3; ++c) x[c] = in_n[t][c] + in_n[t][3 + c] * in_n[t][6];
+              rotate3(x, ln >> 4, xr_n[t]);
+            }
+            static_for<kEncOps>([&](auto q_c) {
+              enc_one(q_c);
+              constexpr int mt = enc_table_slot_at(decltype(q_c)::value);
+              if constexpr (mt >= 0) {
+                f32x2& dst = tbl[mt & 1];
+                asm volatile("s_waitcnt lgkmcnt(0)" : "+v"(dst));
+              }
+            });
+            asm volatile("s_waitcnt vmcnt(10) lgkmcnt(0)" ::: "memory");
+          } else {
+            asm volatile("s_waitcnt vmcnt(0)" ::: "memory");
+          }
+          __builtin_amdgcn_s_barrier();
+          static_for<PipeGeo48::PREFETCH - 1>([&](auto e_c) { pipe.template prologue_read<decltype(e_c)::value>(); });
+          pipe.template bias_prefetch<0>(bias_at(0));
+          pipe.template prologue_read<PipeGeo48::PREFETCH - 1>();
+          pipe.settle();
+#pragma unroll
+          for (int t = 0; t < PT; ++t) { out4[t][0] = 0.0f; out4[t][1] = 0.0f; out4[t][2] = 0.0f; }
+        }
+      } else {
+      if constexpr (TSKIP) {
+        run_stage48x<F, PX, NT - NT_A - 1, KH, 0, (POS_F + (NT_A + 1) * KH) % PX, false, 0, 12, 12, KH, 1>(pipe, hx, no_pe, bias_at(bias_tile + 2 + NT_A), 0u, pacc,
+            [&](auto nt_c, auto s_c) { hidden_op48<F, true, decltype(nt_c)::value + NT_A + 1, decltype(s_c)::value>(pacc, hy); },
+            [&](auto s_c) { hidden_op48<F, true, NT_A, decltype(s_c)::value>(pacc, hy); }, &trk);
+      } else {
+        run_stage48x<F, PX, NT, KH, 0, POS_F, false, 0, 12, 3, KH, 1>(pipe, hx, no_pe, bias_at(bias_tile + 1), 0u, pacc,
+            [&](auto nt_c, auto s_c) { hidden_op48<F, true, decltype(nt_c)::value, decltype(s_c)::value>(pacc, hy); }, sigma_pend, &trk);
+      }
       bias_tile += NT + 1;
       __builtin_amdgcn_sched_barrier(0);
       {
@@ -336,13 +481,6 @@
       __builtin_amdgcn_sched_barrier(0);
       constexpr int POS_D = (POS_F + NT * KH) % PX;
       constexpr int KT_D = KH + KDP;
-      BP8 bg[PT][KH / 2];
-      BP8 ped[PT];
-      typedef float f32x2 __attribute__((ext_vector_type(2)));
-      float ev[2] = {0.0f, 0.0f};
-      f32x2 tbl[2] = {{0.0f, 0.0f}, {0.0f, 0.0f}};
-      unsigned tab_addr_v = 0u, stash_addr_v = 0u;
-      float in_n[PT][7];
       if constexpr (OVX) {
         static_assert(kEncOps <= enc_begin((NT / 2) * KT_D, KT_D), "the view-direction stage has a gap for every encoding op");
         {
@@ -381,44 +519,8 @@
         if constexpr (OVX) {
           constexpr int b = decltype(b_c)::value, w = decltype(w_c)::value;
           constexpr int q0 = enc_begin(b, KT_D), cap = enc_cap(b, KT_D);
-          auto one = [&](auto q_c) {
-            constexpr int qq = decltype(q_c)::value;
-            if constexpr (qq < kEncOps) {
-              constexpr int mt = enc_table_slot_at(qq);
-              constexpr int m = enc_slot_of(qq), u = m % 16, tq = m / 16, e = u % 8, k2 = u / 8;
-              constexpr int kind = enc_kind(u, qq - enc_first(m));
-              const unsigned ta = tab_addr_v, sa = stash_addr_v;
-              if constexpr (mt >= 0) {
-                f32x2& dst = tbl[mt & 1];
-                asm volatile("ds_read_b64 %0, %1 offset:%2" : "=v"(dst) : "v"(ta), "n"((mt % 16) * 16));
-              }
-              const float xc = xr_n[tq][u % 3];
-              float& val = ev[e & 1];
-              const f32x2 entry = tbl[m & 1];
-              if constexpr (kind == kEncMul) asm volatile("v_mul_f32 %0, %1, %2" : "=v"(val) : "v"(xc), "v"(entry[0]));
-              else if constexpr (kind == kEncFract) asm volatile("v_fract_f32 %0, %0" : "+v"(val));
-              else if constexpr (kind == kEncAdd) asm volatile("v_add_f32 %0, %0, %1" : "+v"(val) : "v"(entry[1]));
-              else if constexpr (kind == kEncSin) asm volatile("v_sin_f32 %0, %0" : "+v"(val));
-              else if constexpr (kind == kEncSel) {
-                const unsigned long long im = idm[u < 3 ? u : 0];
-                asm volatile("v_cndmask_b32 %0, %0, %1, %2" : "+v"(val) : "v"(xc), "s"(im));
-              } else if constexpr (kind == kEncCvt) {
-                typedef unsigned u32x4 __attribute__((ext_vector_type(4)));
-                const float lo = ev[0], hi = ev[1];
-                unsigned dw;
-                if constexpr (F == 1) asm volatile("v_cvt_pk_bf16_f32 %0, %1, %2" : "=v"(dw) : "v"(lo), "v"(hi));
-                else asm volatile("v_cvt_pk_f16_f32 %0, %1, %2" : "=v"(dw) : "v"(lo), "v"(hi));
-                u32x4 pw = __builtin_bit_cast(u32x4, encp);
-                pw[e / 2] = dw;
-                encp = __builtin_bit_cast(BP8, pw);
-              } else {
-                const BP8 piece = encp;
-                asm volatile("ds_write_b128 %0, %1 offset:%2" : : "v"(sa), "v"(piece), "n"((tq * KXP + k2) * kPieceBytes));
-              }
-            }
-          };
-          if constexpr (w < 2) one(std::integral_constant<int, q0 + w>{});
-          else if constexpr (w == 2) static_for<cap - 2>([&](auto j_c) { one(std::integral_constant<int, q0 + 2 + decltype(j_c)::value>{}); });
+          if constexpr (w < 2) enc_one(std::integral_constant<int, q0 + w>{});
+          else if constexpr (w == 2) static_for<cap - 2>([&](auto j_c) { enc_one(std::integral_constant<int, q0 + 2 + decltype(j_c)::value>{}); });
         }
       };
       run_stage48x<F, PX, NT / 2, KH, KDP, POS_D, false, 0, 12, 12, (NT - 1) / 2, 1>(pipe, hy, [&](int t, int) { return ped[t]; }, bias_at(bias_tile), 0u, pacc,
@@ -437,6 +539,7 @@
       else pipe.settle();
       asm volatile("s_nop 7\n\ts_nop 1" ::: "memory");
       static_for<9>([&](auto s_c) { constexpr int sv = decltype(s_c)::value; pick_op48(out4[sv / 3][sv % 3], pacc[sv / 3][sv % 3]); });
+      }
     } else {
     {
       BP8 pe[PT][KXP];
diff --git a/dex-nerf_amd/csrc/mlp_geo48.h b/dex-nerf_amd/csrc/mlp_geo48.h
--- a/dex-nerf_amd/csrc/mlp_geo48.h
+++ b/dex-nerf_amd/csrc/mlp_geo48.h
@@ -35,7 +35,10 @@
   const char* base;
   int bias_bytes;
   int total_pieces;
-  CompParams comp;
+  union {
+    CompParams comp;
+    int skip_transparent;
+  };
 };
 
 
@@ -77,6 +80,11 @@
   L.total_bias_tiles = bias;
   L.bias_bytes = round_up(bias * 64, 1024);
   return 0;
+}
+
+constexpr int g48_paper_bias_tiles(int W, int D) { return (W / 16) * D + (W / 16 + 1) + W / 32 + 1; }
+inline bool g48_verdict_words_fit(const NetLayout& L) {
+  return L.use_viewdirs && L.total_bias_tiles == g48_paper_bias_tiles(L.W, L.D) && L.total_bias_tiles * 64 + 8 <= L.bias_bytes;
 }
 
 inline size_t g48_lds_bytes(const NetLayout& L) {
@@ -209,7 +217,7 @@
 
 int launch_pack48(const dn_mlp_desc& d, int precision, const PackPtrs& ptrs, char* region, hipStream_t stream);
 int launch_forward48(const dn_mlp_desc& d, int precision, const FwdParams& p, const char* region, hipStream_t stream,
-                     const CompParams* comp = nullptr, int* composited = nullptr);
+                     const CompParams* comp = nullptr, int* composited = nullptr, int skip_transparent = 0);
 int backward48_entry(const dn_mlp_desc* desc, const void* packed_bwd, const float* g_out, const void* masks, int64_t n_points,
                      void* grads, float grad_scale, hipStream_t stream, const unsigned* partials = nullptr, int n_partials = 0);
 int unpack48_entry(const dn_mlp_desc* desc, int which, const void* native, int64_t n_points, int slot, int width, int kind, float* out,
diff --git a/dex-nerf_amd/csrc/mlp_internal.h b/dex-nerf_amd/csrc/mlp_internal.h
--- a/dex-nerf_amd/csrc/mlp_internal.h
+++ b/dex-nerf_amd/csrc/mlp_internal.h
@@ -10,7 +10,8 @@
 
 int setup_params(const dn_mlp_desc* desc, int precision, const void* packed, FwdParams* p);
 struct CompParams;
-int dispatch_forward(const dn_mlp_desc& d, int precision, FwdParams& p, hipStream_t stream, const CompParams* comp = nullptr, int* composited = nullptr);
+int dispatch_forward(const dn_mlp_desc& d, int precision, FwdParams& p, hipStream_t stream, const CompParams* comp = nullptr, int* composited = nullptr,
+                     int skip_transparent = 0);
 int launch_pack(const NetLayout& L, const PackPtrs& ptrs, void* packed, int precision, hipStream_t stream);
 
 }
diff --git a/dex-nerf_amd/csrc/mlp_stage48.h b/dex-nerf_amd/csrc/mlp_stage48.h
--- a/dex-nerf_amd/csrc/mlp_stage48.h
+++ b/dex-nerf_amd/csrc/mlp_stage48.h
@@ -190,7 +190,7 @@
   template <class B, class W>
   __device__ __forceinline__ void operator()(B, W) const {}
 };
-template <int F, int PX, int NT_OUT, int KH, int KP, int POS0, bool LAST, int PAD, int NOPS, int PEND_N, int PEND_BY, int TRK = 0, class PipeT, class BH,
+template <int F, int PX, int NT_OUT, int KH, int KP, int POS0, bool LAST, int PAD, int NOPS, int PEND_N, int PEND_BY, int TRK = 0, bool PIN = (F == 1 && PX == 2 * kPhasePieces), class PipeT, class BH,
           class BP, class Ops, class Pend, class Hook = XsNoHook>
 __device__ __forceinline__ void run_stage48x(PipeT& pipe, const BH& bh, BP&& bp, unsigned bias_addr, unsigned next_addr, f32x4 (&pacc)[3],
                                              Ops&& ops, Pend&& pend, unsigned* trk = nullptr, Hook&& hook = Hook{}) {
@@ -236,7 +236,7 @@
     static_for<KT>([&](auto k_c) {
       constexpr int k = decltype(k_c)::value;
       constexpr int pos = POS0 + nt * KT + k;
-      pipe.template at_position_xs<PX, pos>();
+      pipe.template at_position_xs<PX, pos, PIN>();
       f32x4 b = {0.0f, 0.0f, 0.0f, 0.0f};
       if constexpr (k == 0) b = pipe.template bias_take<1>();
       constexpr int newer = g48_issued<LAST, POS0 + NT_OUT * KT, PAD>(pos + 1, pos + PipeGeo48::PREFETCH) + ((k == KT - 1) ? 1 : 0);
```

Result: faster. 5.616 million rays/s, median of 6 (+6.4%).
